# geek-ai/MAgent

Hardware: NVIDIA B200
Metric: agent-steps/sec on battle map at 1/2/4/8 B200 vs ref C++ on host cores (higher is better)
Workload: dtype f32

## Files before the change

magent_b200/csrc/backend_cuda.cu:

```cuda
#include <cooperative_groups.h>
#include <cuda_runtime.h>
#include <cuda_fp16.h>
#include <stdio.h>
#include <stdlib.h>
#include <string>
#include <string.h>
#include <atomic>
#include <mutex>
#include <vector>

#include "backend.h"
#if defined(MG_PHASE_TIMING)
namespace mg { __device__ long long mg_phase_clock[8 * 32]; }
#endif
#include "obs_phases.h"

namespace cg = cooperative_groups;

namespace mg {
[[noreturn]] void fatal(const char *fmt, ...);
namespace be {

#define CUDA_CHECK(expr)                                                                          \
    do {                                                                                          \
        cudaError_t _e = (expr);                                                                  \
        if (_e != cudaSuccess) mg::fatal("CUDA error %s at %s:%d (%s)", cudaGetErrorString(_e),   \
                                         __FILE__, __LINE__, #expr);                              \
    } while (0)

static std::atomic<long long> g_launches{0};

enum { ATTR_STEP = 0, ATTR_OBS0 = 1, ATTR_N = 1 + 8, ATTR_MAX_DEVICES = 64 };
static std::mutex g_attr_mu;
static size_t g_attr_smem[ATTR_MAX_DEVICES][ATTR_N];
template <class K>
static void ensure_dynamic_smem(int device, int slot, K kernel, size_t smem) {
    std::lock_guard<std::mutex> lk(g_attr_mu);
    size_t &have = g_attr_smem[device % ATTR_MAX_DEVICES][slot];
    if (smem <= have) return;
    CUDA_CHECK(cudaFuncSetAttribute(kernel, cudaFuncAttributeMaxDynamicSharedMemorySize, (int)smem));
    have = smem;
}

struct Ctx {
    int device = 0, sms = 0;
    cudaStream_t stream = nullptr;
    cudaStream_t copy = nullptr;
    cudaEvent_t ev_wire = nullptr, ev_done = nullptr;
    bool profile = false;
    std::vector<cudaEvent_t> events;
    size_t events_used = 0;
    float *mm_pad = nullptr; size_t mm_pad_n = 0; int mm_stride = 0;
    int4 *obs_hdr = nullptr; size_t obs_hdr_n = 0;
    struct ObsCfg { size_t smem = (size_t)-1; int ctas_per_sm = 1; } obs_cfg[8];
    int *pin_done = nullptr; size_t pin_done_n = 0;
    int *pin_counts = nullptr; size_t pin_counts_n = 0;
    cudaEvent_t ev_counts = nullptr;
    WireMark *wire_slots = nullptr; size_t wire_slots_n = 0;
    WireMark *wire_stream = nullptr; size_t wire_stream_n = 0;
    WireHdr *wire_hdr = nullptr; size_t wire_hdr_n = 0;
    long long *wire_base = nullptr; size_t wire_base_n = 0;
    int *wire_chunk_total = nullptr;
    WireHdr *h_wire_hdr = nullptr; size_t h_wire_hdr_n = 0;
    WireMark *h_wire_marks = nullptr; size_t h_wire_marks_n = 0;
    long long *h_wire_base = nullptr; size_t h_wire_base_n = 0;
    float *h_mm = nullptr; size_t h_mm_n = 0;
    std::vector<cudaEvent_t> wave_events;
    int waves_queued = 0;
    std::vector<cudaEvent_t> dma_events; size_t dma_head = 0, dma_tail = 0;
    bool capturing = false;
    std::vector<cudaGraphExec_t> graphs;
};

static void no_capture(const Ctx *c, const char *what) {
    if (c->capturing) mg::fatal("%s is not possible while a CUDA graph is being captured (run one un-captured step first so that "
                                "every buffer has its size)", what);
}

struct DeviceGuard {
    explicit DeviceGuard(const Ctx *c) { int cur = -1; cudaGetDevice(&cur); if (cur != c->device) CUDA_CHECK(cudaSetDevice(c->device)); }
};

const char *name() { return "cuda-sm_100a"; }

#if defined(MG_PHASE_TIMING)
extern "C" __attribute__((visibility("default"))) void magent_b200_debug_phase_clocks(long long *out) {
    CUDA_CHECK(cudaMemcpyFromSymbol(out, mg::mg_phase_clock, sizeof(long long) * 8 * 32));
}
#endif

int device_count() {
    int n = 0;
    if (cudaGetDeviceCount(&n) != cudaSuccess) { cudaGetLastError(); return 0; }
    return n;
}

Ctx *create(int device, std::string *err) {
    int n = device_count();
    if (n <= 0) { if (err) *err = "cudaGetDeviceCount found no device"; return nullptr; }
    if (device < 0) {
        if (cudaGetDevice(&device) != cudaSuccess) device = 0;
    }
    if (device >= n) { if (err) *err = "device_id out of range"; return nullptr; }
    cudaError_t e = cudaSetDevice(device);
    if (e != cudaSuccess) { if (err) *err = cudaGetErrorString(e); return nullptr; }
    cudaDeviceProp prop;
    CUDA_CHECK(cudaGetDeviceProperties(&prop, device));
    Ctx *c = new Ctx();
    c->device = device;
    c->sms = prop.multiProcessorCount;
    CUDA_CHECK(cudaStreamCreate(&c->stream));
    CUDA_CHECK(cudaStreamCreateWithFlags(&c->copy, cudaStreamNonBlocking));
    CUDA_CHECK(cudaEventCreateWithFlags(&c->ev_wire, cudaEventDisableTiming));
    CUDA_CHECK(cudaEventCreateWithFlags(&c->ev_done, cudaEventDisableTiming));
    CUDA_CHECK(cudaEventCreateWithFlags(&c->ev_counts, cudaEventDisableTiming));
    return c;
}
void destroy(Ctx *c) {
    if (!c) return;
    cudaSetDevice(c->device);
    for (cudaGraphExec_t e : c->graphs) if (e) cudaGraphExecDestroy(e);
    cudaStreamSynchronize(c->stream); cudaStreamSynchronize(c->copy);
    for (cudaEvent_t e : c->events) cudaEventDestroy(e);
    for (cudaEvent_t e : c->wave_events) cudaEventDestroy(e);
    for (cudaEvent_t e : c->dma_events) cudaEventDestroy(e);
    cudaEventDestroy(c->ev_wire); cudaEventDestroy(c->ev_done);
    cudaFree(c->mm_pad); cudaFree(c->obs_hdr);
    cudaFree(c->wire_slots); cudaFree(c->wire_stream); cudaFree(c->wire_hdr); cudaFree(c->wire_base); cudaFree(c->wire_chunk_total);
    cudaEventDestroy(c->ev_counts); cudaFreeHost(c->pin_counts);
    cudaFreeHost(c->pin_done); cudaFreeHost(c->h_wire_hdr); cudaFreeHost(c->h_wire_marks); cudaFreeHost(c->h_wire_base); cudaFreeHost(c->h_mm);
    cudaStreamDestroy(c->stream); cudaStreamDestroy(c->copy);
    delete c;
}
int device_of(const Ctx *c) { return c->device; }
int sm_count(const Ctx *c) { return c->sms; }
void *stream_handle(const Ctx *c) { return (void *)c->stream; }

void *dmalloc(Ctx *c, size_t bytes) { no_capture(c, "a device allocation"); DeviceGuard g(c); void *p = nullptr; CUDA_CHECK(cudaMalloc(&p, bytes ? bytes : 16)); return p; }
void dfree(Ctx *c, void *p) { if (p) { DeviceGuard g(c); cudaFree(p); } }
void dmemset(Ctx *c, void *p, int byte, size_t bytes) { DeviceGuard g(c); CUDA_CHECK(cudaMemsetAsync(p, byte, bytes, c->stream)); }
void h2d(Ctx *c, void *dst, const void *src, size_t bytes) {
    if (!bytes) return;
    no_capture(c, "a blocking host-to-device copy");
    DeviceGuard g(c);
    CUDA_CHECK(cudaMemcpyAsync(dst, src, bytes, cudaMemcpyHostToDevice, c->stream));
    CUDA_CHECK(cudaStreamSynchronize(c->stream));
}
void d2h(Ctx *c, void *dst, const void *src, size_t bytes) {
    if (!bytes) return;
    no_capture(c, "a blocking device-to-host copy");
    DeviceGuard g(c);
    CUDA_CHECK(cudaMemcpyAsync(dst, src, bytes, cudaMemcpyDeviceToHost, c->stream));
    CUDA_CHECK(cudaStreamSynchronize(c->stream));
}
void d2d(Ctx *c, void *dst, const void *src, size_t bytes) {
    if (!bytes) return;
    DeviceGuard g(c);
    CUDA_CHECK(cudaMemcpyAsync(dst, src, bytes, cudaMemcpyDeviceToDevice, c->stream));
}
void *host_alloc(size_t bytes) {
    void *p = nullptr;
    if (cudaHostAlloc(&p, bytes ? bytes : 16, cudaHostAllocPortable) != cudaSuccess) { cudaGetLastError(); return nullptr; }
    return p;
}
void host_free(void *p) { if (p) cudaFreeHost(p); }
bool host_register(void *p, size_t bytes) {
    if (cudaHostRegister(p, bytes, cudaHostRegisterPortable) != cudaSuccess) { cudaGetLastError(); return false; }
    return true;
}
void host_unregister(void *p) { if (cudaHostUnregister(p) != cudaSuccess) cudaGetLastError(); }
bool is_device_ptr(const void *p) {
    if (!p) return false;
    cudaPointerAttributes at;
    if (cudaPointerGetAttributes(&at, p) != cudaSuccess) { cudaGetLastError(); return false; }
    return at.type == cudaMemoryTypeDevice || at.type == cudaMemoryTypeManaged;
}
bool is_pinned_host_ptr(const void *p) {
    if (!p) return false;
    cudaPointerAttributes at;
    if (cudaPointerGetAttributes(&at, p) != cudaSuccess) { cudaGetLastError(); return false; }
    return at.type == cudaMemoryTypeHost;
}
void sync(Ctx *c) { no_capture(c, "a synchronisation"); DeviceGuard g(c); CUDA_CHECK(cudaStreamSynchronize(c->stream)); CUDA_CHECK(cudaStreamSynchronize(c->copy)); }
long long launch_count() { return g_launches.load(); }
void profile_enable(Ctx *c, bool on) { c->profile = on; c->events_used = 0; }
static void profile_pair(Ctx *c, cudaEvent_t *e0, cudaEvent_t *e1) {
    if (c->events_used + 2 > c->events.size()) {
        for (int i = 0; i < 64; ++i) { cudaEvent_t e; CUDA_CHECK(cudaEventCreate(&e)); c->events.push_back(e); }
    }
    *e0 = c->events[c->events_used]; *e1 = c->events[c->events_used + 1];
    c->events_used += 2;
}
void profile_read(Ctx *c, double *ms, long long *n) {
    DeviceGuard g(c);
    double total = 0.0;
    for (size_t i = 0; i + 1 < c->events_used; i += 2) {
        CUDA_CHECK(cudaEventSynchronize(c->events[i + 1]));
        float t = 0;
        CUDA_CHECK(cudaEventElapsedTime(&t, c->events[i], c->events[i + 1]));
        total += t;
    }
    *ms = total; *n = (long long)(c->events_used / 2);
}

bool capture_begin(Ctx *c) {
    DeviceGuard guard(c);
    CUDA_CHECK(cudaStreamSynchronize(c->stream));
    CUDA_CHECK(cudaStreamBeginCapture(c->stream, cudaStreamCaptureModeRelaxed));
    c->capturing = true;
    return true;
}
int capture_end(Ctx *c) {
    DeviceGuard guard(c);
    cudaGraph_t g = nullptr;
    c->capturing = false;
    CUDA_CHECK(cudaStreamEndCapture(c->stream, &g));
    cudaGraphExec_t exec = nullptr;
    CUDA_CHECK(cudaGraphInstantiate(&exec, g, 0));
    CUDA_CHECK(cudaGraphDestroy(g));
    c->graphs.push_back(exec);
    return (int)c->graphs.size() - 1;
}
bool capturing(const Ctx *c) { return c->capturing; }
void graph_launch(Ctx *c, int id) {
    DeviceGuard guard(c);
    if (id < 0 || id >= (int)c->graphs.size() || !c->graphs[id]) mg::fatal("invalid graph id %d", id);
    CUDA_CHECK(cudaGraphLaunch(c->graphs[id], c->stream));
}
void graph_destroy_all(Ctx *c) {
    DeviceGuard guard(c);
    for (cudaGraphExec_t e : c->graphs) if (e) cudaGraphExecDestroy(e);
    c->graphs.clear();
}

static void post_launch(const char *what) {
    ++g_launches;
    cudaError_t e = cudaGetLastError();
    if (e != cudaSuccess) mg::fatal("kernel launch failed (%s): %s", what, cudaGetErrorString(e));
}

__device__ __forceinline__ int block_excl_scan(int v, int &total) {
    __shared__ int warp_sums[32];
    __shared__ int block_total;
    const int lane = threadIdx.x & 31, wid = threadIdx.x >> 5, nw = (blockDim.x + 31) >> 5;
    int incl = v;
#pragma unroll
    for (int d = 1; d < 32; d <<= 1) {
        int t = __shfl_up_sync(0xffffffffu, incl, d);
        if (lane >= d) incl += t;
    }
    if (lane == 31) warp_sums[wid] = incl;
    __syncthreads();
    if (wid == 0) {
        int w = lane < nw ? warp_sums[lane] : 0;
        int wi = w;
#pragma unroll
        for (int d = 1; d < 32; d <<= 1) {
            int t = __shfl_up_sync(0xffffffffu, wi, d);
            if (lane >= d) wi += t;
        }
        if (lane < nw) warp_sums[lane] = wi - w;
        if (lane == 31) block_total = wi;
    }
    __syncthreads();
    int excl = incl - v + warp_sums[wid];
    total = block_total;
    __syncthreads();
    return excl;
}

struct CtaCtx {
    GroupEnum *enum_smem;
    MG_HD GroupEnum *enums() { return enum_smem; }
    MG_HD bool is_cta_leader() const {
#if defined(__CUDA_ARCH__)
        return threadIdx.x == 0;
#else
        return true;
#endif
    }
    MG_HD void sync_cta() {
#if defined(__CUDA_ARCH__)
        __syncthreads();
#endif
    }
    int *flag_smem;
    MG_HD int *flags(ArenaHdr *) { return flag_smem; }
    int cnt[MG_N_COUNTERS];
    MG_HD void add_count(const EngineDev &, int kind, long long v) { cnt[kind] += (int)v; }
    int *cnt_smem;
    MG_HD void flush_counts(const EngineDev &E) {
#if defined(__CUDA_ARCH__)
#pragma unroll
        for (int k = 0; k < MG_N_COUNTERS; ++k) {
            int v = cnt[k];
            cnt[k] = 0;
#pragma unroll
            for (int d = 16; d > 0; d >>= 1) v += __shfl_xor_sync(0xffffffffu, v, d);
            if (v && (threadIdx.x & 31) == 0) atomicAdd(&cnt_smem[k], v);
        }
        __syncthreads();
        if (threadIdx.x < MG_N_COUNTERS) {
            const int v = cnt_smem[threadIdx.x];
            cnt_smem[threadIdx.x] = 0;
            if (v) atomicAdd((unsigned long long *)&E.counters[threadIdx.x], (unsigned long long)v);
        }
#endif
    }
    MG_HD int tid() const {
#if defined(__CUDA_ARCH__)
        return threadIdx.x;
#else
        return 0;
#endif
    }
    MG_HD int nth() const {
#if defined(__CUDA_ARCH__)
        return blockDim.x;
#else
        return 1;
#endif
    }
    MG_HD void sync() {
#if defined(__CUDA_ARCH__)
        __syncthreads();
#endif
    }
    template <class P, class Em>
    MG_HD int scan(int n, P pred, Em emit) {
#if defined(__CUDA_ARCH__)
        int running = 0;
        for (int tile = 0; tile < n; tile += blockDim.x) {
            int i = tile + threadIdx.x;
            int p = i < n ? pred(i) : 0;
            int tot;
            int ex = block_excl_scan(p, tot);
            if (p) emit(i, running + ex);
            running += tot;
        }
        return running;
#else
        return 0;
#endif
    }
};

struct GridCtx {
    GroupEnum *enum_smem;
    MG_HD GroupEnum *enums() { return enum_smem; }
    MG_HD bool is_cta_leader() const {
#if defined(__CUDA_ARCH__)
        return threadIdx.x == 0;
#else
        return true;
#endif
    }
    MG_HD void sync_cta() {
#if defined(__CUDA_ARCH__)
        __syncthreads();
#endif
    }
    int *scratch;
    int parity;
    MG_HD int *flags(ArenaHdr *hdr) { return hdr->changed; }
    int cnt[MG_N_COUNTERS];
    MG_HD void add_count(const EngineDev &, int kind, long long v) { cnt[kind] += (int)v; }
    MG_HD void flush_counts(const EngineDev &E) {
#if defined(__CUDA_ARCH__)
#pragma unroll
        for (int k = 0; k < MG_N_COUNTERS; ++k) {
            int v = cnt[k];
            cnt[k] = 0;
#pragma unroll
            for (int d = 16; d > 0; d >>= 1) v += __shfl_xor_sync(0xffffffffu, v, d);
            if (v && (threadIdx.x & 31) == 0) atomicAdd((unsigned long long *)&E.counters[k], (unsigned long long)v);
        }
#endif
    }
    MG_HD int tid() const {
#if defined(__CUDA_ARCH__)
        return blockIdx.x * blockDim.x + threadIdx.x;
#else
        return 0;
#endif
    }
    MG_HD int nth() const {
#if defined(__CUDA_ARCH__)
        return gridDim.x * blockDim.x;
#else
        return 1;
#endif
    }
    MG_HD void sync() {
#if defined(__CUDA_ARCH__)
        cg::this_grid().sync();
#endif
    }
    template <class P, class Em>
    MG_HD int scan(int n, P pred, Em emit) {
#if defined(__CUDA_ARCH__)
        const int nb = gridDim.x, bid = blockIdx.x;
        const int L = (n + nb - 1) / nb;
        const int lo = min(n, bid * L), hi = min(n, lo + L);
        int cnt = 0;
        for (int i = lo + threadIdx.x; i < hi; i += blockDim.x) cnt += pred(i);
        int cta_total;
        block_excl_scan(cnt, cta_total);
        int *sc = scratch + (parity & 1) * 4096;
        parity ^= 1;
        if (threadIdx.x == 0) sc[bid] = cta_total;
        cg::this_grid().sync();
        int below = 0, all = 0;
        for (int b = threadIdx.x; b < nb; b += blockDim.x) { int v = sc[b]; all += v; if (b < bid) below += v; }
        int base, total;
        block_excl_scan(below, base);
        block_excl_scan(all, total);
        int running = base;
        for (int tile = lo; tile < hi; tile += blockDim.x) {
            int i = tile + threadIdx.x;
            int p = i < hi ? pred(i) : 0;
            int tot;
            int ex = block_excl_scan(p, tot);
            if (p) emit(i, running + ex);
            running += tot;
        }
        return total;
#else
        return 0;
#endif
    }
};

__device__ __forceinline__ void load_engine(EngineDev *sE, const EngineDev *gE) {
    const int *src = (const int *)gE;
    int *dst = (int *)sE;
    for (int i = threadIdx.x; i < (int)(sizeof(EngineDev) / sizeof(int)); i += blockDim.x) dst[i] = src[i];
    __syncthreads();
}

constexpr int STEP_THREADS = 1024;
constexpr int GRID_THREADS = 512;

static size_t step_scratch_bytes(int cap_total, int max_body) {
    return (size_t)cap_total * (9 * 4 + 4 * (size_t)max_body) + (((size_t)cap_total + 15) & ~(size_t)15);
}

__device__ __forceinline__ void step_scratch_to_smem(EngineDev *sE, unsigned char *base) {
    const size_t n = (size_t)sE->cap_total;
    int *p = (int *)base;
    sE->att_rank = p; p += n;  sE->tgt = p; p += n;       sE->in_head = p; p += n;  sE->in_next = p; p += n;
    sE->death = p; p += n;
    sE->mv_nx = p; sE->jv = p; p += n;
    sE->mv_ny = p; sE->sh_head = p; p += n;
    sE->mv_key = (unsigned *)p; sE->sh_next = p; p += n;
    sE->hp_fin = (float *)p; sE->att_agent = p; p += n;
    sE->cl_next = p; sE->sh_first = p; p += n * sE->max_body;
    sE->mv_state = (unsigned char *)p;
    sE->scratch_stride = 0;
}

__global__ void __launch_bounds__(STEP_THREADS) step_kernel_cta(const EngineDev *gE, StepArgs S, int scratch_in_smem) {
    extern __shared__ __align__(16) unsigned char step_smem[];
    __shared__ EngineDev sE;
    load_engine(&sE, gE);
    if (scratch_in_smem) {
        if (threadIdx.x == 0) step_scratch_to_smem(&sE, step_smem);
        __syncthreads();
    }
    __shared__ int relax_flags[3];
    __shared__ int counter_sums[MG_N_COUNTERS];
    __shared__ GroupEnum enum_store[2];
    if (threadIdx.x < MG_N_COUNTERS) counter_sums[threadIdx.x] = 0;
    CtaCtx c;
    c.flag_smem = relax_flags;
    c.cnt_smem = counter_sums;
    c.enum_smem = enum_store;
    for (int k = 0; k < MG_N_COUNTERS; ++k) c.cnt[k] = 0;
    for (int a = blockIdx.x; a < sE.A; a += gridDim.x) run_step(c, sE, S, a);
}

__global__ void __launch_bounds__(STEP_THREADS) step_kernel_grid(const EngineDev *gE, StepArgs S) {
    __shared__ EngineDev sE;
    load_engine(&sE, gE);
    __shared__ GroupEnum enum_store[2];
    GridCtx c;
    c.scratch = sE.team_scratch;
    c.parity = 0;
    c.enum_smem = enum_store;
    for (int k = 0; k < MG_N_COUNTERS; ++k) c.cnt[k] = 0;
    for (int a = 0; a < sE.A; ++a) run_step(c, sE, S, a);
}

__global__ void __launch_bounds__(STEP_THREADS) cull_kernel_cta(const EngineDev *gE, unsigned curmask) {
    __shared__ EngineDev sE;
    load_engine(&sE, gE);
    CtaCtx c;
    c.flag_smem = nullptr;
    c.cnt_smem = nullptr;
    c.enum_smem = nullptr;
    for (int a = blockIdx.x; a < sE.A; a += gridDim.x) run_cull(c, sE, curmask, a);
}

__global__ void __launch_bounds__(STEP_THREADS) cull_kernel_grid(const EngineDev *gE, unsigned curmask) {
    __shared__ EngineDev sE;
    load_engine(&sE, gE);
    GridCtx c;
    c.scratch = sE.team_scratch;
    c.parity = 0;
    c.enum_smem = nullptr;
    for (int a = 0; a < sE.A; ++a) run_cull(c, sE, curmask, a);
}

static const int GRID_MODE_THRESHOLD = 32768;

static int step_block_size(int sms, int arenas, int max_agents) {
    if (arenas >= 2 * sms) return 256;
    if (max_agents >= 768) return 1024;
    return max_agents >= 384 ? 512 : 256;
}

static int coop_grid(const Ctx *c, const void *kernel) {
    int per_sm = 0;
    CUDA_CHECK(cudaOccupancyMaxActiveBlocksPerMultiprocessor(&per_sm, kernel, GRID_THREADS, 0));
    if (per_sm < 1) mg::fatal("cooperative kernel does not fit on an SM");
    int g = per_sm * c->sms;
    return g > 4096 ? 4096 : g;
}

void launch_step(Ctx *c, const EngineDev *dE, const EngineDev &hE, const StepArgs &S, int max_agents) {
    DeviceGuard guard(c);
    const int g_sms = c->sms;
    if (max_agents > GRID_MODE_THRESHOLD) {
        int grid = coop_grid(c, (const void *)step_kernel_grid);
        StepArgs s = S;
        void *args[] = {(void *)&dE, (void *)&s};
        CUDA_CHECK(cudaLaunchCooperativeKernel((const void *)step_kernel_grid, dim3(grid), dim3(GRID_THREADS), args, 0, c->stream));
        post_launch("step_kernel_grid");
    } else {
        const size_t sbytes = step_scratch_bytes(hE.cap_total, hE.max_body);
        static const int smem_pref = getenv("MAGENT_B200_STEP_SMEM") ? atoi(getenv("MAGENT_B200_STEP_SMEM")) : -1;
        const bool in_smem = sbytes <= 200 * 1024 && smem_pref != 0;
        int threads = step_block_size(g_sms, hE.A, max_agents);
        size_t smem = 0;
        if (in_smem) {
            smem = sbytes;
            threads = max_agents >= 768 ? (hE.A > g_sms ? 512 : 1024) : (max_agents >= 384 ? 512 : 256);
            ensure_dynamic_smem(c->device, ATTR_STEP, step_kernel_cta, smem);
        }
        static const int threads_pref = getenv("MAGENT_B200_STEP_THREADS") ? atoi(getenv("MAGENT_B200_STEP_THREADS")) : 0;
        if (threads_pref >= 32 && threads_pref <= STEP_THREADS) threads = threads_pref & ~31;
        int per_sm = 1;
        CUDA_CHECK(cudaOccupancyMaxActiveBlocksPerMultiprocessor(&per_sm, step_kernel_cta, threads, smem));
        if (per_sm < 1) per_sm = 1;
        int grid = hE.A < per_sm * g_sms ? hE.A : per_sm * g_sms;
        step_kernel_cta<<<grid, threads, smem, c->stream>>>(dE, S, in_smem ? 1 : 0);
        post_launch("step_kernel_cta");
    }
}

void launch_cull(Ctx *c, const EngineDev *dE, const EngineDev &hE, unsigned curmask, int max_agents) {
    DeviceGuard guard(c);
    const int g_sms = c->sms;
    if (max_agents > GRID_MODE_THRESHOLD) {
        int grid = coop_grid(c, (const void *)cull_kernel_grid);
        void *args[] = {(void *)&dE, (void *)&curmask};
        CUDA_CHECK(cudaLaunchCooperativeKernel((const void *)cull_kernel_grid, dim3(grid), dim3(GRID_THREADS), args, 0, c->stream));
        post_launch("cull_kernel_grid");
    } else {
        int grid = hE.A < 8 * g_sms ? hE.A : 8 * g_sms;
        static const int cull_pref = getenv("MAGENT_B200_CULL_THREADS") ? atoi(getenv("MAGENT_B200_CULL_THREADS")) : 0;
        int threads = max_agents >= 768 ? 512 : step_block_size(g_sms, hE.A, max_agents);
        if (cull_pref >= 32 && cull_pref <= STEP_THREADS) threads = cull_pref & ~31;
        cull_kernel_cta<<<grid, threads, 0, c->stream>>>(dE, curmask);
        post_launch("cull_kernel_cta");
    }
}

__global__ void __launch_bounds__(1024) offsets_kernel(const EngineDev *gE) {
    const int g = blockIdx.x;
    const int A = gE->A;
    const int *n = gE->n + (size_t)g * A;
    int *off = gE->off + (size_t)g * (A + 1);
    int running = 0;
    for (int tile = 0; tile < A; tile += blockDim.x) {
        int a = tile + threadIdx.x;
        int v = a < A ? n[a] : 0;
        int tot;
        int ex = block_excl_scan(v, tot);
        if (a < A) off[a] = running + ex;
        running += tot;
    }
    if (threadIdx.x == 0) off[A] = running;
}

void launch_offsets(Ctx *c, const EngineDev *dE, const EngineDev &hE) {
    DeviceGuard guard(c);
    offsets_kernel<<<hE.G, 1024, 0, c->stream>>>(dE);
    post_launch("offsets_kernel");
}

__device__ __forceinline__ int locate_arena(const int *off, int A, int idx) {
    int lo = 0, hi = A;
    while (hi - lo > 1) {
        int mid = (lo + hi) >> 1;
        if (off[mid] <= idx) lo = mid; else hi = mid;
    }
    return lo;
}

__global__ void __launch_bounds__(256) info_kernel(const EngineDev *gE, unsigned curmask, int kind, int g,
                                                   void *buf, int n_total, int chunks_per_arena) {
    const EngineDev &E = *gE;
    const int *off = E.off + (size_t)g * (E.A + 1);
    const AgentSoA &s = E.grp[g].soa[(curmask >> g) & 1u];
    const int a = blockIdx.x / chunks_per_arena;
    const int i = (blockIdx.x - a * chunks_per_arena) * blockDim.x + threadIdx.x;
    const int o0 = off[a];
    const int o = o0 + i;
    if (i < off[a + 1] - o0 && o < n_total) {
        const long gi = (long)a * E.grp[g].cap + i;
        switch (kind) {
            case INFO_ID: ((int *)buf)[o] = s.id[gi]; break;
            case INFO_POS: ((int2 *)buf)[o] = make_int2(s.x[gi], s.y[gi]); break;
            case INFO_ALIVE: ((unsigned char *)buf)[o] = (s.flags[gi] & FLAG_DEAD) ? 0 : 1; break;
            case INFO_REWARD: ((float *)buf)[o] = s.next_reward[gi] + E.hdr[a].grp_reward[g]; break;
            case INFO_HP: ((float *)buf)[o] = s.hp[gi]; break;
            case INFO_ACTION_SCATTER: s.act[gi] = ((const int *)buf)[o]; break;
        }
    }
}

void launch_info(Ctx *c, const EngineDev *dE, const EngineDev &hE, unsigned curmask, int kind, int group, void *buf, int n_total) {
    DeviceGuard guard(c);
    const int cap = hE.grp[group].cap;
    const int threads = cap >= 256 ? 256 : ((cap + 31) & ~31);
    const int cpa = (cap + threads - 1) / threads;
    info_kernel<<<(unsigned)((size_t)hE.A * cpa), threads, 0, c->stream>>>(dE, curmask, kind, group, buf, n_total, cpa);
    post_launch("info_kernel");
}

__device__ __forceinline__ unsigned long long splitmix64(unsigned long long x) {
    x += 0x9E3779B97F4A7C15ull;
    x = (x ^ (x >> 30)) * 0xBF58476D1CE4E5B9ull;
    x = (x ^ (x >> 27)) * 0x94D049BB133111EBull;
    return x ^ (x >> 31);
}

__global__ void __launch_bounds__(256) random_actions_kernel(const EngineDev *gE, unsigned curmask, int g,
                                                             unsigned long long seed, int n_total, int chunks_per_arena) {
    const EngineDev &E = *gE;
    const int *off = E.off + (size_t)g * (E.A + 1);
    const AgentSoA &s = E.grp[g].soa[(curmask >> g) & 1u];
    const unsigned na = (unsigned)E.grp[g].n_action;
    seed += (unsigned long long)E.counters[CNT_STEPS] * 0xA24BAED4963EE407ull;
    const int a = blockIdx.x / chunks_per_arena;
    const int i = (blockIdx.x - a * chunks_per_arena) * blockDim.x + threadIdx.x;
    const int o0 = off[a];
    const int o = o0 + i;
    if (i < off[a + 1] - o0 && o < n_total)
        s.act[(long)a * E.grp[g].cap + i] = (int)((splitmix64(seed ^ ((unsigned long long)o * 0xD1342543DE82EF95ull)) >> 33) % na);
}

void launch_random_actions(Ctx *c, const EngineDev *dE, const EngineDev &hE, unsigned curmask, int group,
                           unsigned long long seed, int n_total) {
    DeviceGuard guard(c);
    const int cap = hE.grp[group].cap;
    const int threads = cap >= 256 ? 256 : ((cap + 31) & ~31);
    const int cpa = (cap + threads - 1) / threads;
    random_actions_kernel<<<(unsigned)((size_t)hE.A * cpa), threads, 0, c->stream>>>(dE, curmask, group, seed, n_total, cpa);
    post_launch("random_actions_kernel");
}

__global__ void __launch_bounds__(256) minimap_small_kernel(const EngineDev *gE, unsigned curmask, int og, float *mm_val, int stride) {
    extern __shared__ int hist[];
    __shared__ int counted_s;
    const EngineDev &E = *gE;
    const int ag = blockIdx.x;
    const int a = ag / E.G, j = ag - a * E.G;
    const int vw = E.grp[og].view_w, vh = E.grp[og].view_h, cells = vw * vh;
    const int n = E.n[j * E.A + a];
    for (int k = threadIdx.x; k < cells; k += blockDim.x) hist[k] = 0;
    if (threadIdx.x == 0) counted_s = 0;
    __syncthreads();
    const GroupDev &G = E.grp[j];
    const AgentSoA &s = G.soa[(curmask >> j) & 1u];
    const int scale_h = (E.H + vh - 1) / vh, scale_w = (E.W + vw - 1) / vw;
    const bool skip_absorbed = E.grp[og].can_absorb != 0;
    int counted = 0;
    for (int i = threadIdx.x; i < n; i += blockDim.x) {
        const long gi = (long)a * G.cap + i;
        if (skip_absorbed && (s.flags[gi] & FLAG_ABSORBED)) continue;
        atomicAdd(&hist[(s.y[gi] / scale_h) * vw + s.x[gi] / scale_w], 1);
        ++counted;
    }
#pragma unroll
    for (int d = 16; d > 0; d >>= 1) counted += __shfl_xor_sync(0xffffffffu, counted, d);
    if ((threadIdx.x & 31) == 0 && counted) atomicAdd(&counted_s, counted);
    __syncthreads();
    const int tot = counted_s;
    float *out = mm_val + (size_t)a * stride + (size_t)j * cells;
    for (int k = threadIdx.x; k < cells; k += blockDim.x)
        out[k] = tot ? (float)hist[k] / (float)tot : __int_as_float((int)0xFFC00000u);
}

__global__ void __launch_bounds__(256) obs_prepare_kernel(const EngineDev *gE, unsigned curmask, int og, int chunk) {
    extern __shared__ int hist[];
    const EngineDev &E = *gE;
    const int ag = blockIdx.y;
    const int a = ag / E.G, j = ag - a * E.G;
    const int vw = E.grp[og].view_w, vh = E.grp[og].view_h, cells = vw * vh;
    const int n = E.n[j * E.A + a];
    const int lo = blockIdx.x * chunk;
    if (lo >= n) return;
    const int hi = min(n, lo + chunk);
    for (int k = threadIdx.x; k < cells; k += blockDim.x) hist[k] = 0;
    __syncthreads();
    const GroupDev &G = E.grp[j];
    const AgentSoA &s = G.soa[(curmask >> j) & 1u];
    const int scale_h = (E.H + vh - 1) / vh, scale_w = (E.W + vw - 1) / vw;
    const bool skip_absorbed = E.grp[og].can_absorb != 0;
    int counted = 0;
    for (int i = lo + threadIdx.x; i < hi; i += blockDim.x) {
        long gi = (long)a * G.cap + i;
        if (skip_absorbed && (s.flags[gi] & FLAG_ABSORBED)) continue;
        atomicAdd(&hist[(s.y[gi] / scale_h) * vw + s.x[gi] / scale_w], 1);
        ++counted;
    }
    if (counted) atomicAdd(&E.mm_total[ag], counted);
    __syncthreads();
    int *out = E.mm_count + (size_t)ag * cells;
    for (int k = threadIdx.x; k < cells; k += blockDim.x)
        if (hist[k]) atomicAdd(&out[k], hist[k]);
}

__global__ void __launch_bounds__(256) minimap_norm_kernel(const EngineDev *gE, int og, float *mm_val, int total, int stride) {
    const EngineDev &E = *gE;
    const int cells = E.grp[og].view_w * E.grp[og].view_h;
    for (int k = blockIdx.x * blockDim.x + threadIdx.x; k < total; k += gridDim.x * blockDim.x) {
        int ag = k / cells;
        const int tot = E.mm_total[ag];
        const int a = ag / E.G;
        mm_val[(size_t)a * stride + (k - a * E.G * cells)] = tot ? (float)E.mm_count[k] / (float)tot : __int_as_float((int)0xFFC00000u);
    }
}

void launch_obs_prepare(Ctx *c, const EngineDev *dE, const EngineDev &hE, unsigned curmask, int og, float *mm_val) {
    if (!mm_val) return;
    DeviceGuard guard(c);
    const int g_sms = c->sms;
    const int cells = hE.grp[og].view_w * hE.grp[og].view_h;
    const int total = hE.A * hE.G * cells;
    int cap_max = 0;
    for (int g = 0; g < hE.G; ++g) cap_max = cap_max > hE.grp[g].cap ? cap_max : hE.grp[g].cap;
    c->mm_stride = (hE.G * cells + 3) & ~3;
    const size_t need = (size_t)hE.A * c->mm_stride;
    if (need > c->mm_pad_n) {
        no_capture(c, "growing the minimap buffer");
        if (c->mm_pad) { CUDA_CHECK(cudaStreamSynchronize(c->stream)); CUDA_CHECK(cudaStreamSynchronize(c->copy)); cudaFree(c->mm_pad); }
        CUDA_CHECK(cudaMalloc(&c->mm_pad, need * sizeof(float)));
        CUDA_CHECK(cudaMemsetAsync(c->mm_pad, 0, need * sizeof(float), c->stream));
        c->mm_pad_n = need;
    }
    if (cap_max <= 8192 && (size_t)cells * sizeof(int) <= 48 * 1024) {
        minimap_small_kernel<<<hE.A * hE.G, 256, cells * sizeof(int), c->stream>>>(dE, curmask, og, c->mm_pad, c->mm_stride);
        post_launch("minimap_small_kernel");
        return;
    }
    CUDA_CHECK(cudaMemsetAsync(hE.mm_count, 0, (size_t)total * 4, c->stream));
    CUDA_CHECK(cudaMemsetAsync(hE.mm_total, 0, (size_t)hE.A * hE.G * 4, c->stream));
    const int chunk = 4096;
    dim3 grid((cap_max + chunk - 1) / chunk, hE.A * hE.G);
    obs_prepare_kernel<<<grid, 256, cells * sizeof(int), c->stream>>>(dE, curmask, og, chunk);
    post_launch("obs_prepare_kernel");
    int g2 = (total + 255) / 256;
    if (g2 > 8 * g_sms) g2 = 8 * g_sms;
    minimap_norm_kernel<<<g2, 256, 0, c->stream>>>(dE, og, c->mm_pad, total, c->mm_stride);
    post_launch("minimap_norm_kernel");
}

#ifndef OBS_TA_N
#define OBS_TA_N 4
#endif
#ifndef OBS_ABLATE
#define OBS_ABLATE 0
#endif

template <typename T> struct ObsOut;
template <> struct ObsOut<float> {
    static constexpr int TA = OBS_TA_N;
    static __device__ __forceinline__ float cv(float v) { return v; }
};
template <> struct ObsOut<__half> {
    static constexpr int TA = 2 * OBS_TA_N;
    static __device__ __forceinline__ __half cv(float v) {
        if (v != v) {
            const unsigned u = __float_as_uint(v);
            unsigned short r = (unsigned short)(0x7c00u + ((u & 0x7fffffu) >> 13));
            if (r == 0x7c00u) ++r;
            return __ushort_as_half((unsigned short)(r | ((u >> 16) & 0x8000u)));
        }
        return __float2half_rn(v);
    }
};

struct ObsParams {
    int A, W, H, G, C;
    int vw, vh, cells, rec, F;
    int ox, oy;
    int scale_w, scale_h, minimap;
    int cap, embedding, n_action, n_total;
    const unsigned char *mask;
    const int *off;
    const unsigned char *kind_plane;
    const float *hpn_plane;
    int kpad, kw;
    long kplane;
    int chunk;
    int turn, body_w, body_l;
    const unsigned char *dir;
    const int *x, *y, *id, *act;
    const float *last_reward;
    const float *mm;
    int mm_stride;
    const int4 *hdr;
    void *view, *feature;
    int mm_ch[MG_MAX_GROUPS];
    int grp_ch[MG_MAX_GROUPS];
};

__device__ __forceinline__ uint32_t smem_u32(const void *p) { return (uint32_t)__cvta_generic_to_shared(p); }

template <typename T>
__global__ void __launch_bounds__(256) obs_headers_kernel(ObsParams P, int4 *hdr, int chunks_per_arena) {
    extern __shared__ __align__(16) unsigned char hdr_smem[];
    T *rows = (T *)hdr_smem;
    const int a = blockIdx.x / chunks_per_arena;
    const int i0 = (blockIdx.x - a * chunks_per_arena) * blockDim.x;
    const int o0 = P.off[a], n_a = P.off[a + 1] - o0;
    if (i0 >= n_a) return;
    int cnt = min((int)blockDim.x, n_a - i0);
    cnt = min(cnt, P.n_total - (o0 + i0));
    if (cnt <= 0) return;
    const int total = cnt * P.F;
    for (int q = threadIdx.x; q < total; q += blockDim.x) rows[q] = ObsOut<T>::cv(0.0f);
    __syncthreads();
    if ((int)threadIdx.x < cnt) {
        const int i = i0 + threadIdx.x;
        const long gi = (long)a * P.cap + i;
        const int x = P.x[gi], y = P.y[gi];
        const int self_cell = P.minimap ? (y / P.scale_h) * P.vw + x / P.scale_w : -1;
        const int heading = P.turn ? (int)P.dir[gi] : 0;
        hdr[o0 + i] = make_int4(x, y, a, (self_cell & 0xffff) | (heading << 16));
        T *f = rows + (size_t)threadIdx.x * P.F;
        unsigned id = (unsigned)P.id[gi];
        const int nbits = min(P.embedding, 31);
        id &= nbits >= 32 ? 0xffffffffu : ((1u << nbits) - 1u);
        while (id) {
            const int bit = __ffs(id) - 1;
            f[bit] = ObsOut<T>::cv(1.0f);
            id &= id - 1;
        }
        T *g = f + P.embedding;
        const int act = P.act[gi];
        if (act >= 0 && act < P.n_action) g[act] = ObsOut<T>::cv(1.0f);
        g[P.n_action] = ObsOut<T>::cv(P.last_reward[gi]);
        if (P.minimap) {
            g[P.n_action + 1] = ObsOut<T>::cv((float)x / (float)P.W);
            g[P.n_action + 2] = ObsOut<T>::cv((float)y / (float)P.H);
        }
    }
    __syncthreads();
    T *out = (T *)P.feature + (size_t)(o0 + i0) * P.F;
    if (sizeof(T) == 4 && ((((size_t)out) & 15) == 0)) {
        const int v4 = total >> 2;
        for (int q = threadIdx.x; q < v4; q += blockDim.x) ((float4 *)out)[q] = ((const float4 *)rows)[q];
        for (int q = (v4 << 2) + threadIdx.x; q < total; q += blockDim.x) out[q] = rows[q];
    } else {
        for (int q = threadIdx.x; q < total; q += blockDim.x) out[q] = rows[q];
    }
}

#ifndef OBS_MIN_CTAS
#define OBS_MIN_CTAS 8
#endif
#ifndef OBS_CHUNK
#define OBS_CHUNK 4
#endif
template <typename T, int NIT, bool TURN>
__global__ void __launch_bounds__(32 * ObsOut<T>::TA, OBS_MIN_CTAS * OBS_TA_N / ObsOut<T>::TA)
obs_render_kernel(const __grid_constant__ ObsParams P) {
    const int n_total = min(P.n_total, __ldg(P.off + P.A));
    constexpr int OBS_TA = ObsOut<T>::TA;
    constexpr int OBS_THREADS = 32 * OBS_TA;
    extern __shared__ __align__(128) unsigned char smem_raw[];
    T *buf = (T *)smem_raw;
    int2 *lut = (int2 *)(buf + OBS_TA * P.rec);
    __shared__ int n_in_s;
    const int lane = threadIdx.x & 31, warp = threadIdx.x >> 5;

    const int lut_stride = (P.cells + 1) & ~1;
    if (warp == 0) {
        int k = 0;
        for (int base = 0; base < P.cells; base += 32) {
            const int cell = base + lane;
            const bool in = cell < P.cells && P.mask[cell];
            const unsigned bal = __ballot_sync(0xffffffffu, in);
            if (in) {
                const int vy = cell / P.vw, vx = cell - vy * P.vw;
                const int q = k + __popc(bal & ((1u << lane) - 1u));
                if (!TURN) lut[q] = make_int2(cell * P.C, (P.oy + vy) * P.kw + P.ox + vx);
                else {
                    for (int d = 0; d < 4; ++d) {
                        int rx = 0, ry = 0, dx, dy;
                        if (d == DIR_SOUTH) { rx = P.body_w - 1; ry = P.body_l - 1; }
                        else if (d == DIR_WEST) ry = P.body_w - 1;
                        else if (d == DIR_EAST) rx = P.body_l - 1;
                        const int ex = P.ox + vx, ey = P.oy + vy;
                        if (d == DIR_NORTH) { dx = ex; dy = ey; }
                        else if (d == DIR_SOUTH) { dx = -ex; dy = -ey; }
                        else if (d == DIR_WEST) { dx = ey; dy = -ex; }
                        else { dx = -ey; dy = ex; }
                        lut[d * lut_stride + q] = make_int2(cell * P.C, (ry + dy) * P.kw + rx + dx);
                    }
                }
            }
            k += __popc(bal);
        }
        if (lane == 0) n_in_s = k;
    }
    __syncthreads();
    const int n_in = n_in_s;
    const int n_tiles = (n_total + OBS_TA - 1) / OBS_TA;
    constexpr bool LUT_REGS = NIT <= 4 && !TURN;
    int2 lreg[LUT_REGS ? NIT : 1];
    if (LUT_REGS) {
#pragma unroll
        for (int it = 0; it < (LUT_REGS ? NIT : 1); ++it) lreg[it] = it * 32 + lane < n_in ? lut[it * 32 + lane] : make_int2(-1, 0);
    }
    auto lutv = [&](int it, int hd) -> int2 {
        if (TURN) return it * 32 + lane < n_in ? lut[hd * lut_stride + it * 32 + lane] : make_int2(-1, 0);
        return LUT_REGS ? lreg[LUT_REGS ? it : 0] : (it * 32 + lane < n_in ? lut[it * 32 + lane] : make_int2(-1, 0));
    };
    auto plane_base = [&](const int4 &h) -> long { return h.z * P.kplane + (long)(h.y + P.kpad) * P.kw + h.x + P.kpad; };

    auto load_kinds = [&](const int4 &h, bool on, int (&kd)[NIT]) {
        const unsigned char *kp = P.kind_plane + plane_base(h);
        const int hd = TURN ? (h.w >> 16) & 3 : 0;
#pragma unroll
        for (int it = 0; it < NIT; ++it) {
            const int2 l = lutv(it, hd);
            kd[it] = (on && l.x >= 0 && !(OBS_ABLATE & 1)) ? __ldg(kp + l.y) : 0;
        }
    };
    unsigned long long chpack = 0ull;
#pragma unroll
    for (int j = 0; j < MG_MAX_GROUPS; ++j) chpack |= (unsigned long long)(P.grp_ch[j] & 0xff) << (8 * j);
    auto mark = [&](T *px, int t, float hp, bool on) {
        const bool agent = kind_is_agent(t);
        const int ch = agent ? (int)((chpack >> (8 * kind_group(t))) & 0xffull) : (t == KIND_FOOD ? 1 : 0);
        px[ch] = ObsOut<T>::cv(on ? 1.0f : 0.0f);
        if (agent) px[ch + 1] = ObsOut<T>::cv(on ? hp : 0.0f);
    };

    const int chunk = P.chunk;
    const int chunk_jump = ((int)gridDim.x - 1) * chunk;
    auto next_tile = [&](int t) -> int { return ((t + 1) % chunk) ? t + 1 : t + 1 + chunk_jump; };
    int tile = blockIdx.x * chunk;
    int tile1 = next_tile(tile), tile2 = next_tile(tile1);
    const int tile_end = n_tiles;
    const int4 zero4 = make_int4(0, 0, 0, 0);
    int4 hA = zero4, hA1 = zero4;
    int kind[NIT];
    int rec_arena = -1, prev_hd = 0, prev_self = -1;
    unsigned prev_kinds[(NIT + 3) / 4];
#pragma unroll
    for (int q = 0; q < (NIT + 3) / 4; ++q) prev_kinds[q] = 0u;
    float self_orig = 0.0f;
    bool prev_tail = false;
    {
        const int o0 = tile * OBS_TA + warp, o1 = tile1 * OBS_TA + warp;
        const bool on0 = tile < tile_end && o0 < n_total;
        if (on0) hA = P.hdr[o0];
        if (o1 < n_total) hA1 = P.hdr[o1];
        load_kinds(hA, on0, kind);
    }
    for (; tile < tile_end; tile = tile1, tile1 = tile2, tile2 = next_tile(tile2)) {
        const int t0 = tile * OBS_TA;
        const int cnt = min(OBS_TA, n_total - t0);
        const bool active = warp < cnt;
        const int a = hA.z;
        const float *hpnp = P.hpn_plane + plane_base(hA);
        const int hd = TURN ? (hA.w >> 16) & 3 : 0;
        float thp[NIT];
#pragma unroll
        for (int it = 0; it < NIT; ++it) {
            thp[it] = 0.0f;
            if (kind_is_agent(kind[it])) thp[it] = (kind[it] & KIND_FULL) ? 1.0f : __ldg(hpnp + lutv(it, hd).y);
        }
        int kind1[NIT];
        const long o1 = (long)tile1 * OBS_TA + warp;
        load_kinds(hA1, o1 < n_total, kind1);
        int4 hA2 = zero4;
        {
            const long o2 = (long)tile2 * OBS_TA + warp;
            if (o2 < n_total) hA2 = P.hdr[o2];
        }
        if (threadIdx.x == 0) asm volatile("cp.async.bulk.wait_group.read 0;" ::: "memory");
        __syncthreads();
        if (active && !(OBS_ABLATE & 2)) {
            T *dst = buf + warp * P.rec;
            const int self = (int)(short)(hA.w & 0xffff);
            if (a != rec_arena) {
                if (sizeof(T) == 4) {
                    float *w = (float *)dst;
                    const int n = P.rec;
                    const int head = min(n, (int)((4u - ((unsigned)(warp * P.rec) & 3u)) & 3u));
                    const int body = (n - head) >> 2;
                    if (lane < head) w[lane] = 0.0f;
                    float4 *w4 = (float4 *)(w + head);
                    const float4 z = make_float4(0.f, 0.f, 0.f, 0.f);
                    for (int q = lane; q < body; q += 32) w4[q] = z;
                    const int tail0 = head + (body << 2);
                    if (tail0 + lane < n) w[tail0 + lane] = 0.0f;
                } else {
                    for (int q = lane; q < P.rec; q += 32) dst[q] = ObsOut<T>::cv(0.0f);
                }
                __syncwarp();
                if (P.minimap) {
                    const float *rows = P.mm + (size_t)a * P.mm_stride;
                    for (int j = 0; j < P.G; ++j) {
                        T *d = dst + P.mm_ch[j];
                        for (int cell = lane; cell < P.cells; cell += 32) d[cell * P.C] = ObsOut<T>::cv(__ldg(rows + j * P.cells + cell));
                    }
                }
                rec_arena = a;
                __syncwarp();
            } else {
#pragma unroll
                for (int it = 0; it < NIT; ++it) {
                    const int t = (prev_kinds[it >> 2] >> ((it & 3) * 8)) & 0xff;
                    if (t != 0) mark(dst + lutv(it, prev_hd).x, t, 0.0f, false);
                }
                if (prev_tail) {
                    for (int k = NIT * 32 + lane; k < n_in; k += 32) {
                        T *px = dst + lut[(TURN ? prev_hd * lut_stride : 0) + k].x;
                        for (int ch = 0; ch < P.C; ++ch) {
                            bool mm_ch = false;
                            for (int j = 0; j < P.G; ++j) mm_ch |= P.minimap && ch == P.mm_ch[j];
                            if (!mm_ch) px[ch] = ObsOut<T>::cv(0.0f);
                        }
                    }
                }
                if (P.minimap && lane < P.G && prev_self >= 0) dst[prev_self * P.C + P.mm_ch[lane]] = ObsOut<T>::cv(self_orig);
                __syncwarp();
            }
            if (P.minimap && lane < P.G) {
                const float v = __ldg(P.mm + (size_t)a * P.mm_stride + lane * P.cells + self);
                self_orig = v;
                if (v == v) dst[self * P.C + P.mm_ch[lane]] = ObsOut<T>::cv(v + 1.0f);
            }
            prev_self = self;
            prev_hd = hd;
#pragma unroll
            for (int q = 0; q < (NIT + 3) / 4; ++q) prev_kinds[q] = 0u;
#pragma unroll
            for (int it = 0; it < NIT; ++it) {
                const int t = kind[it];
                prev_kinds[it >> 2] |= (unsigned)t << ((it & 3) * 8);
                if (t != 0) mark(dst + lutv(it, hd).x, t, thp[it], true);
            }
            prev_tail = false;
            const unsigned char *kindp = P.kind_plane + plane_base(hA);
            for (int k = NIT * 32 + lane; k < n_in; k += 32) {
                const int2 l = lut[(TURN ? hd * lut_stride : 0) + k];
                const int t = __ldg(kindp + l.y);
                if (t != 0) { mark(dst + l.x, t, kind_is_agent(t) ? ((t & KIND_FULL) ? 1.0f : __ldg(hpnp + l.y)) : 0.0f, true); }
                prev_tail = true;
            }
        }
        asm volatile("fence.proxy.async.shared::cta;" ::: "memory");
        __syncthreads();
        T *gout = (T *)P.view + (size_t)t0 * P.rec;
        const unsigned bytes = (unsigned)cnt * (unsigned)P.rec * (unsigned)sizeof(T);
        if ((bytes & 15u) == 0 && (((size_t)gout) & 15) == 0) {
            if (threadIdx.x == 0 && !(OBS_ABLATE & 8)) {
                asm volatile("cp.async.bulk.global.shared::cta.bulk_group [%0], [%1], %2;"
                             :: "l"(gout), "r"(smem_u32(buf)), "r"(bytes) : "memory");
                asm volatile("cp.async.bulk.commit_group;" ::: "memory");
            }
        } else {
            for (int q = threadIdx.x; q < cnt * P.rec; q += OBS_THREADS) gout[q] = buf[q];
            __syncthreads();
        }
        hA = hA1; hA1 = hA2;
#pragma unroll
        for (int it = 0; it < NIT; ++it) kind[it] = kind1[it];
    }
    if (threadIdx.x == 0) asm volatile("cp.async.bulk.wait_group 0;" ::: "memory");
}

template <typename T, int NIT, bool TURN>
static void launch_obs_typed(Ctx *c, int cfg_slot, const EngineDev &hE, ObsParams &P, int n_total,
                             bool with_headers = true, bool headers_only = false) {
    const int g_sms = c->sms;
    constexpr int TA = ObsOut<T>::TA;
    constexpr int THREADS = 32 * TA;
    const size_t tile_bytes = (size_t)TA * P.rec * sizeof(T);
    const size_t smem = tile_bytes + (size_t)(P.turn ? 4 : 1) * ((P.cells + 1) & ~1) * sizeof(int2);
    if (smem > 227 * 1024) mg::fatal("observation record too large for the render kernel (%zu bytes of shared memory)", smem);
    const int tiles = (n_total + TA - 1) / TA;
    if ((size_t)n_total > c->obs_hdr_n) {
        no_capture(c, "growing the observation header table");
        if (c->obs_hdr) { CUDA_CHECK(cudaStreamSynchronize(c->stream)); cudaFree(c->obs_hdr); }
        c->obs_hdr_n = (size_t)n_total + n_total / 4 + 64;
        CUDA_CHECK(cudaMalloc(&c->obs_hdr, c->obs_hdr_n * sizeof(int4)));
    }
    P.hdr = c->obs_hdr;
    if (with_headers) {
        int threads = 256;
        while (threads > 32 && (size_t)threads * P.F * sizeof(T) > 48 * 1024) threads >>= 1;
        const size_t hsm = (size_t)threads * P.F * sizeof(T);
        if (hsm > 48 * 1024) mg::fatal("feature row too long for the header kernel (%d elements)", P.F);
        const int cpa = (P.cap + threads - 1) / threads;
        obs_headers_kernel<T><<<(unsigned)((size_t)P.A * cpa), threads, hsm, c->stream>>>(P, c->obs_hdr, cpa);
        post_launch("obs_headers_kernel");
    }
    if (headers_only) return;
    Ctx::ObsCfg &cfg = c->obs_cfg[cfg_slot];
    ensure_dynamic_smem(c->device, ATTR_OBS0 + cfg_slot, obs_render_kernel<T, NIT, TURN>, smem);
    if (smem != cfg.smem) {
        CUDA_CHECK(cudaOccupancyMaxActiveBlocksPerMultiprocessor(&cfg.ctas_per_sm, obs_render_kernel<T, NIT, TURN>, THREADS, smem));
        if (cfg.ctas_per_sm < 1) cfg.ctas_per_sm = 1;
        cfg.smem = smem;
    }
    const int ctas_per_sm = cfg.ctas_per_sm;
    const int grid = tiles < ctas_per_sm * g_sms ? tiles : ctas_per_sm * g_sms;
    P.chunk = tiles / (ctas_per_sm * g_sms);
    if (P.chunk < 1) P.chunk = 1;
    const int max_chunk = sizeof(T) == 2 ? 2 * OBS_CHUNK : OBS_CHUNK;
    if (P.chunk > max_chunk) P.chunk = max_chunk;
    cudaEvent_t e0 = nullptr, e1 = nullptr;
    const bool timed = c->profile && !c->capturing;
    if (timed) { profile_pair(c, &e0, &e1); CUDA_CHECK(cudaEventRecord(e0, c->stream)); }
    obs_render_kernel<T, NIT, TURN><<<grid, THREADS, smem, c->stream>>>(P);
    post_launch("obs_render_kernel");
    if (timed) CUDA_CHECK(cudaEventRecord(e1, c->stream));
}

static void fill_obs_params(Ctx *c, const EngineDev &hE, const ObsArgs &O, const float *mm_val, int n_total, ObsParams &P) {
    const int g = O.group;
    const GroupDev &G = hE.grp[g];
    memset(&P, 0, sizeof P);
    P.A = hE.A; P.W = hE.W; P.H = hE.H; P.G = hE.G; P.C = hE.n_channel;
    P.vw = G.view_w; P.vh = G.view_h; P.cells = G.view_w * G.view_h; P.rec = P.cells * P.C; P.F = G.feature_size;
    P.ox = G.view_xoff + G.view_x1; P.oy = G.view_yoff + G.view_y1;
    P.scale_w = (hE.W + G.view_w - 1) / G.view_w; P.scale_h = (hE.H + G.view_h - 1) / G.view_h;
    P.minimap = mm_val != nullptr;
    P.cap = G.cap; P.embedding = hE.embedding_size; P.n_action = G.n_action; P.n_total = n_total;
    P.mask = G.view_mask;
    P.off = hE.off + (size_t)g * (hE.A + 1);
    P.kind_plane = hE.kind; P.hpn_plane = hE.hpn; P.kpad = hE.kpad; P.kw = hE.kw; P.kplane = hE.kplane;
    const AgentSoA &s = G.soa[(O.curmask >> g) & 1u];
    P.x = s.x; P.y = s.y; P.id = s.id; P.act = s.act; P.last_reward = s.last_reward; P.dir = s.dir;
    P.turn = hE.turn_mode; P.body_w = G.body_w; P.body_l = G.body_l;
    P.mm = mm_val ? c->mm_pad : nullptr; P.mm_stride = mm_val ? c->mm_stride : 0;
    P.view = O.view; P.feature = O.feature;
    const int stride = 2 + (hE.minimap_mode ? 1 : 0);
    for (int j = 0; j < hE.G; ++j) {
        int rel = j - g; if (rel < 0) rel += hE.G;
        const int ch = hE.channel_base + rel * stride;
        P.mm_ch[j] = ch + 2;
        P.grp_ch[j] = ch;
    }
}

static void launch_obs_dispatch(Ctx *c, const EngineDev &hE, const ObsArgs &O, ObsParams &P, int n_total, bool with_headers, bool headers_only) {
    const bool small_view = hE.grp[O.group].view_count <= 4 * 32;
    if (hE.turn_mode) {
        if (O.half) launch_obs_typed<__half, 8, true>(c, 0, hE, P, n_total, with_headers, headers_only);
        else launch_obs_typed<float, 8, true>(c, 1, hE, P, n_total, with_headers, headers_only);
    } else if (O.half) {
        if (small_view) launch_obs_typed<__half, 4, false>(c, 2, hE, P, n_total, with_headers, headers_only);
        else launch_obs_typed<__half, 8, false>(c, 3, hE, P, n_total, with_headers, headers_only);
    } else {
        if (small_view) launch_obs_typed<float, 4, false>(c, 4, hE, P, n_total, with_headers, headers_only);
        else launch_obs_typed<float, 8, false>(c, 5, hE, P, n_total, with_headers, headers_only);
    }
}

void launch_obs(Ctx *c, const EngineDev *, const EngineDev &hE, const ObsArgs &O, const float *mm_val, int n_total) {
    DeviceGuard guard(c);
    ObsParams P;
    fill_obs_params(c, hE, O, mm_val, n_total, P);
    launch_obs_dispatch(c, hE, O, P, n_total, true, false);
}

__global__ void __launch_bounds__(256) done_reduce_kernel(const EngineDev *gE, int *out) {
    __shared__ int all_s;
    if (threadIdx.x == 0) all_s = 1;
    __syncthreads();
    int all = 1;
    for (int a = threadIdx.x; a < gE->A; a += blockDim.x) all &= gE->done[a] & 1;
    if (!all) all_s = 0;
    __syncthreads();
    if (threadIdx.x == 0) *out = all_s;
}

void read_done(Ctx *c, const EngineDev &hE, int *done_words) {
    no_capture(c, "env_step with a host `done`");
    DeviceGuard guard(c);
    if ((size_t)hE.A > c->pin_done_n) {
        if (c->pin_done) cudaFreeHost(c->pin_done);
        c->pin_done_n = (size_t)hE.A + 64;
        CUDA_CHECK(cudaHostAlloc((void **)&c->pin_done, c->pin_done_n * sizeof(int), cudaHostAllocDefault));
    }
    CUDA_CHECK(cudaMemcpyAsync(c->pin_done, hE.done, (size_t)hE.A * sizeof(int), cudaMemcpyDeviceToHost, c->stream));
    CUDA_CHECK(cudaStreamSynchronize(c->stream));
    memcpy(done_words, c->pin_done, (size_t)hE.A * sizeof(int));
}

void counts_fetch_begin(Ctx *c, const int *dev_off, size_t n_ints) {
    no_capture(c, "the asynchronous count fetch");
    DeviceGuard guard(c);
    if (n_ints > c->pin_counts_n) {
        if (c->pin_counts) { CUDA_CHECK(cudaStreamSynchronize(c->stream)); cudaFreeHost(c->pin_counts); }
        c->pin_counts_n = n_ints + 64;
        CUDA_CHECK(cudaHostAlloc((void **)&c->pin_counts, c->pin_counts_n * sizeof(int), cudaHostAllocDefault));
    }
    CUDA_CHECK(cudaMemcpyAsync(c->pin_counts, dev_off, n_ints * sizeof(int), cudaMemcpyDeviceToHost, c->stream));
    CUDA_CHECK(cudaEventRecord(c->ev_counts, c->stream));
}
const int *counts_fetch_wait(Ctx *c) {
    DeviceGuard guard(c);
    CUDA_CHECK(cudaEventSynchronize(c->ev_counts));
    return c->pin_counts;
}

void launch_done_to_device(Ctx *c, const EngineDev *dE, const EngineDev &, int *dev_done) {
    DeviceGuard guard(c);
    done_reduce_kernel<<<1, 256, 0, c->stream>>>(dE, dev_done);
    post_launch("done_reduce_kernel");
}

__global__ void __launch_bounds__(256) obs_wire_kernel(const __grid_constant__ ObsParams P, WireHdr *whdr, WireMark *slots,
                                                       int slot_stride, int *chunk_total) {
    extern __shared__ __align__(16) unsigned char wire_smem[];
    int2 *lut = (int2 *)wire_smem;
    __shared__ int n_in_s;
    const int lane = threadIdx.x & 31, warp = threadIdx.x >> 5;
    const int lut_stride = (P.cells + 1) & ~1;
    if (warp == 0) {
        int k = 0;
        for (int base = 0; base < P.cells; base += 32) {
            const int cell = base + lane;
            const bool in = cell < P.cells && P.mask[cell];
            const unsigned bal = __ballot_sync(0xffffffffu, in);
            if (in) {
                const int vy = cell / P.vw, vx = cell - vy * P.vw;
                const int q = k + __popc(bal & ((1u << lane) - 1u));
                if (!P.turn) lut[q] = make_int2(cell * P.C, (P.oy + vy) * P.kw + P.ox + vx);
                else {
                    for (int d = 0; d < 4; ++d) {
                        int rx = 0, ry = 0, dx, dy;
                        if (d == DIR_SOUTH) { rx = P.body_w - 1; ry = P.body_l - 1; }
                        else if (d == DIR_WEST) ry = P.body_w - 1;
                        else if (d == DIR_EAST) rx = P.body_l - 1;
                        const int ex = P.ox + vx, ey = P.oy + vy;
                        if (d == DIR_NORTH) { dx = ex; dy = ey; }
                        else if (d == DIR_SOUTH) { dx = -ex; dy = -ey; }
                        else if (d == DIR_WEST) { dx = ey; dy = -ex; }
                        else { dx = -ey; dy = ex; }
                        lut[d * lut_stride + q] = make_int2(cell * P.C, (ry + dy) * P.kw + rx + dx);
                    }
                }
            }
            k += __popc(bal);
        }
        if (lane == 0) n_in_s = k;
    }
    __syncthreads();
    const int n_in = n_in_s;
    const int warps = gridDim.x * (blockDim.x >> 5);
    for (int o = blockIdx.x * (blockDim.x >> 5) + warp; o < P.n_total; o += warps) {
        const int4 h = P.hdr[o];
        const long pb = h.z * P.kplane + (long)(h.y + P.kpad) * P.kw + h.x + P.kpad;
        const unsigned char *kp = P.kind_plane + pb;
        const float *hpnp = P.hpn_plane + pb;
        const int2 *l = lut + (P.turn ? ((h.w >> 16) & 3) * lut_stride : 0);
        WireMark *row = slots + (size_t)o * slot_stride;
        int running = 0;
        for (int base = 0; base < n_in; base += 32) {
            const int k = base + lane;
            int t = 0;
            int2 lk = make_int2(0, 0);
            if (k < n_in) { lk = l[k]; t = __ldg(kp + lk.y); }
            const unsigned bal = __ballot_sync(0xffffffffu, t != 0);
            if (t != 0) {
                WireMark m;
                if (t == KIND_WALL) { m.off = (unsigned)lk.x; m.val = 0.0f; }
                else if (t == KIND_FOOD) { m.off = (unsigned)lk.x + 1u; m.val = 0.0f; }
                else { m.off = (unsigned)(lk.x + P.grp_ch[kind_group(t)]) | WIRE_HAS_HP; m.val = (t & KIND_FULL) ? 1.0f : __ldg(hpnp + lk.y); }
                row[running + __popc(bal & ((1u << lane) - 1u))] = m;
            }
            running += __popc(bal);
        }
        if (lane == 0) {
            WireHdr w;
            w.arena = h.z;
            w.self_cell = (unsigned short)(h.w & 0xffff);
            w.count = (unsigned short)running;
            whdr[o] = w;
            if (running) atomicAdd(&chunk_total[o / WIRE_CHUNK], running);
        }
    }
}

__global__ void __launch_bounds__(1024) wire_scan_kernel(const int *chunk_total, long long *base, int n_chunks) {
    __shared__ long long carry_s;
    if (threadIdx.x == 0) carry_s = 0;
    __syncthreads();
    for (int tile = 0; tile < n_chunks; tile += blockDim.x) {
        const int cidx = tile + threadIdx.x;
        const int v = cidx < n_chunks ? chunk_total[cidx] : 0;
        int tot;
        const int ex = block_excl_scan(v, tot);
        const long long carry = carry_s;
        if (cidx < n_chunks) base[cidx] = carry + ex;
        __syncthreads();
        if (threadIdx.x == 0) carry_s = carry + tot;
        __syncthreads();
    }
    if (threadIdx.x == 0) base[n_chunks] = carry_s;
}

__global__ void __launch_bounds__(256) wire_compact_kernel(const WireHdr *whdr, const WireMark *slots, int slot_stride,
                                                           const long long *base, WireMark *stream, int n_total, int n_chunks) {
    __shared__ int off_s[WIRE_CHUNK];
    __shared__ unsigned short cnt_s[WIRE_CHUNK];
    const int lane = threadIdx.x & 31, warp = threadIdx.x >> 5, nw = blockDim.x >> 5;
    for (int ch = blockIdx.x; ch < n_chunks; ch += gridDim.x) {
        const int o0 = ch * WIRE_CHUNK, cnt_obs = min(WIRE_CHUNK, n_total - o0);
        int running = 0;
        for (int tile = 0; tile < WIRE_CHUNK; tile += blockDim.x) {
            const int i = tile + threadIdx.x;
            const int v = i < cnt_obs ? (int)whdr[o0 + i].count : 0;
            int tot;
            const int ex = block_excl_scan(v, tot);
            off_s[i] = running + ex;
            cnt_s[i] = (unsigned short)v;
            running += tot;
        }
        __syncthreads();
        WireMark *dst = stream + base[ch];
        for (int i = warp; i < cnt_obs; i += nw) {
            const int n = cnt_s[i], off = off_s[i];
            const WireMark *src = slots + (size_t)(o0 + i) * slot_stride;
            for (int k = lane; k < n; k += 32) dst[off + k] = src[k];
        }
        __syncthreads();
    }
}

template <class T>
static void grow_dev(Ctx *c, T *&p, size_t &have, size_t need) {
    if (need <= have) return;
    if (p) { CUDA_CHECK(cudaStreamSynchronize(c->stream)); CUDA_CHECK(cudaStreamSynchronize(c->copy)); cudaFree(p); }
    have = need + need / 4 + 64;
    CUDA_CHECK(cudaMalloc((void **)&p, have * sizeof(T)));
}
template <class T>
static void grow_pinned(Ctx *c, T *&p, size_t &have, size_t need) {
    if (need <= have) return;
    if (p) { CUDA_CHECK(cudaStreamSynchronize(c->copy)); cudaFreeHost(p); }
    have = need + need / 2 + 1024;
    CUDA_CHECK(cudaHostAlloc((void **)&p, have * sizeof(T), cudaHostAllocDefault));
}

void obs_wire_begin(Ctx *c, const EngineDev *, const EngineDev &hE, const ObsArgs &O, const float *mm_val, int n_total,
                    WireDesc *out) {
    no_capture(c, "an observation into host memory");
    DeviceGuard guard(c);
    ObsParams P;
    fill_obs_params(c, hE, O, mm_val, n_total, P);
    launch_obs_dispatch(c, hE, O, P, n_total, true, true);
    const int n_in = hE.grp[O.group].view_count;
    const int n_chunks = (n_total + WIRE_CHUNK - 1) / WIRE_CHUNK;
    grow_dev(c, c->wire_slots, c->wire_slots_n, (size_t)n_total * n_in);
    grow_dev(c, c->wire_hdr, c->wire_hdr_n, (size_t)n_total);
    {
        size_t have = c->wire_base_n;
        grow_dev(c, c->wire_base, c->wire_base_n, (size_t)n_chunks + 1);
        if (c->wire_base_n != have) {
            if (c->wire_chunk_total) cudaFree(c->wire_chunk_total);
            CUDA_CHECK(cudaMalloc((void **)&c->wire_chunk_total, c->wire_base_n * sizeof(int)));
        }
    }
    CUDA_CHECK(cudaMemsetAsync(c->wire_chunk_total, 0, (size_t)n_chunks * sizeof(int), c->stream));
    {
        const size_t smem = (size_t)(P.turn ? 4 : 1) * ((P.cells + 1) & ~1) * sizeof(int2);
        if (smem > 48 * 1024) mg::fatal("view too large for the wire kernel (%zu bytes of shared memory)", smem);
        int grid = (n_total + 7) / 8;
        if (grid > 8 * c->sms) grid = 8 * c->sms;
        obs_wire_kernel<<<grid, 256, smem, c->stream>>>(P, c->wire_hdr, c->wire_slots, n_in, c->wire_chunk_total);
        post_launch("obs_wire_kernel");
        wire_scan_kernel<<<1, 1024, 0, c->stream>>>(c->wire_chunk_total, c->wire_base, n_chunks);
        post_launch("wire_scan_kernel");
    }
    grow_pinned(c, c->h_wire_base, c->h_wire_base_n, (size_t)n_chunks + 1);
    CUDA_CHECK(cudaMemcpyAsync(c->h_wire_base, c->wire_base, ((size_t)n_chunks + 1) * sizeof(long long), cudaMemcpyDeviceToHost, c->stream));
    CUDA_CHECK(cudaEventRecord(c->ev_done, c->stream));
    if (mm_val) {
        grow_pinned(c, c->h_mm, c->h_mm_n, (size_t)hE.A * c->mm_stride);
        CUDA_CHECK(cudaMemcpyAsync(c->h_mm, c->mm_pad, (size_t)hE.A * c->mm_stride * sizeof(float), cudaMemcpyDeviceToHost, c->stream));
    }
    grow_pinned(c, c->h_wire_hdr, c->h_wire_hdr_n, (size_t)n_total);
    CUDA_CHECK(cudaEventSynchronize(c->ev_done));
    const long long total_marks = c->h_wire_base[n_chunks];
    grow_dev(c, c->wire_stream, c->wire_stream_n, (size_t)total_marks + 1);
    grow_pinned(c, c->h_wire_marks, c->h_wire_marks_n, (size_t)total_marks + 1);
    {
        int grid = n_chunks < 8 * c->sms ? n_chunks : 8 * c->sms;
        wire_compact_kernel<<<grid, 256, 0, c->stream>>>(c->wire_hdr, c->wire_slots, n_in, c->wire_base, c->wire_stream, n_total, n_chunks);
        post_launch("wire_compact_kernel");
    }
    CUDA_CHECK(cudaEventRecord(c->ev_wire, c->stream));
    CUDA_CHECK(cudaStreamWaitEvent(c->copy, c->ev_wire, 0));
    int cpw = (n_chunks + 7) / 8;
    if (cpw < 4) cpw = 4;
    const int n_waves = (n_chunks + cpw - 1) / cpw;
    while ((int)c->wave_events.size() < n_waves) {
        cudaEvent_t e; CUDA_CHECK(cudaEventCreateWithFlags(&e, cudaEventDisableTiming)); c->wave_events.push_back(e);
    }
    for (int q = 0; q < n_waves; ++q) {
        const int half = (n_waves + 1) / 2;
        const int w = (q & 1) ? half + (q >> 1) : (q >> 1);
        out->wave_order[q] = w;
        const int c0 = w * cpw, c1 = (c0 + cpw < n_chunks) ? c0 + cpw : n_chunks;
        const size_t o0 = (size_t)c0 * WIRE_CHUNK, o1 = (size_t)c1 * WIRE_CHUNK < (size_t)n_total ? (size_t)c1 * WIRE_CHUNK : (size_t)n_total;
        CUDA_CHECK(cudaMemcpyAsync(c->h_wire_hdr + o0, c->wire_hdr + o0, (o1 - o0) * sizeof(WireHdr), cudaMemcpyDeviceToHost, c->copy));
        const long long m0 = c->h_wire_base[c0], m1 = c->h_wire_base[c1];
        if (m1 > m0) CUDA_CHECK(cudaMemcpyAsync(c->h_wire_marks + m0, c->wire_stream + m0, (size_t)(m1 - m0) * sizeof(WireMark), cudaMemcpyDeviceToHost, c->copy));
        CUDA_CHECK(cudaEventRecord(c->wave_events[w], c->copy));
    }
    c->waves_queued = n_waves;
    out->hdr = c->h_wire_hdr; out->marks = c->h_wire_marks; out->chunk_base = c->h_wire_base;
    out->mm = mm_val ? c->h_mm : nullptr; out->mm_stride = mm_val ? c->mm_stride : 0;
    out->n_total = n_total; out->n_chunks = n_chunks; out->n_waves = n_waves; out->chunks_per_wave = cpw;
}

void obs_wire_wait(Ctx *c, int wave) {
    DeviceGuard guard(c);
    CUDA_CHECK(cudaEventSynchronize(c->wave_events[wave]));
}

void dma_d2h_async(Ctx *c, void *dst, const void *src, size_t bytes) {
    DeviceGuard guard(c);
    CUDA_CHECK(cudaMemcpyAsync(dst, src, bytes, cudaMemcpyDeviceToHost, c->copy));
    if (c->dma_events.size() < 64) {
        while (c->dma_events.size() < 64) { cudaEvent_t e; CUDA_CHECK(cudaEventCreateWithFlags(&e, cudaEventDisableTiming)); c->dma_events.push_back(e); }
    }
    if (c->dma_tail - c->dma_head >= c->dma_events.size()) {
        CUDA_CHECK(cudaEventSynchronize(c->dma_events[c->dma_head % c->dma_events.size()]));
        ++c->dma_head;
    }
    CUDA_CHECK(cudaEventRecord(c->dma_events[c->dma_tail % c->dma_events.size()], c->copy));
    ++c->dma_tail;
}

void dma_wait(Ctx *c, int keep_in_flight) {
    DeviceGuard guard(c);
    while ((long long)(c->dma_tail - c->dma_head) > (long long)keep_in_flight) {
        CUDA_CHECK(cudaEventSynchronize(c->dma_events[c->dma_head % c->dma_events.size()]));
        ++c->dma_head;
    }
}

}
}
```

magent_b200/csrc/dev_types.h:

```cpp
#pragma once
#include <stdint.h>
#include "hd.h"

namespace mg {

enum { MG_MAX_GROUPS = 8, MG_MAX_RULES = 64, MG_MAX_PROG = 16, MG_MAX_RECV = 4, MG_MAX_IN = 4, MG_MAX_ALLQ = 16 };
enum { MG_N_COUNTERS = 8 };
enum Counter { CNT_AGENT_STEPS = 0, CNT_ATTACKS, CNT_HITS, CNT_KILLS, CNT_STARVED,
               CNT_MOVES_OK, CNT_MOVES_BLOCKED, CNT_STEPS };

enum : int { OCC_EMPTY = -1, OCC_WALL = -2, OCC_FOOD = -3 };
enum : int { TGT_NONE = -1, TGT_FOOD = -3 };
enum : int { KIND_EMPTY = 0, KIND_WALL = 1, KIND_GROUP0 = 2, KIND_FOOD = 255 };
enum : int { KIND_FULL = 0x40, KIND_GROUP_MASK = 0x3f };
MG_HD unsigned char kind_agent(int g, bool full_hp) { return (unsigned char)((KIND_GROUP0 + g) | (full_hp ? KIND_FULL : 0)); }
MG_HD bool kind_is_agent(int t) { return t >= KIND_GROUP0 && t != KIND_FOOD; }
MG_HD int kind_group(int t) { return (t & KIND_GROUP_MASK) - KIND_GROUP0; }
enum : int { RANK_NONE = -1, DEATH_NEVER = 0x7fffffff, DEATH_BEFORE = -1 };
enum : unsigned { MVKEY_NONE = 0xffffffffu };

enum : unsigned char { FLAG_DEAD = 1, FLAG_ABSORBED = 2 };
enum : unsigned char { MV_NONE = 0, MV_OOB = 1, MV_STATIC_FAIL = 2, MV_PENDING_FAIL = 3, MV_OK = 4, MV_ABSORBED = 5, MV_SKIPPED = 6 };

enum EventOp : unsigned char { OP_AND = 0, OP_OR, OP_NOT, OP_KILL, OP_AT, OP_IN, OP_COLLIDE, OP_ATTACK,
                               OP_DIE, OP_IN_A_LINE, OP_ALIGN, OP_NULL };

MG_HD int code_make(int g, int i) { return (g << 24) | i; }
MG_HD int code_group(int c) { return c >> 24; }
MG_HD int code_index(int c) { return c & 0xffffff; }

enum { DIR_EAST = 0, DIR_SOUTH = 1, DIR_WEST = 2, DIR_NORTH = 3 };

struct AgentSoA {
    int *x, *y;
    float *hp;
    int *act;
    int *id;
    float *next_reward, *last_reward;
    int *op_obj;
    unsigned char *last_op;
    unsigned char *flags;
    unsigned char *dir;
};

struct GroupDev {
    int body_w, body_l;
    float max_hp, damage, step_recover, kill_supply;
    float eat_ability, food_supply;
    float step_reward, kill_reward, dead_penalty, attack_penalty;
    int attack_in_group;
    int can_absorb;
    int view_w, view_h, view_x1, view_y1;
    int view_count;
    int view_xoff, view_yoff;
    int att_xoff, att_yoff;
    int n_move, attack_base, n_action, n_attack;
    int channel;
    int feature_size;
    const int *move_dx, *move_dy;
    const int *att_dx, *att_dy;
    const unsigned char *view_mask;
    int cap;
    int foff;
    AgentSoA soa[2];
    int *ev_rank;
};

struct ArenaHdr {
    uint32_t rng;
    uint32_t rng_next;
    int done;
    int n_attack;
    int any_dead;
    int changed[3];
    unsigned char rule_trig[MG_MAX_RULES];
    float grp_reward[MG_MAX_GROUPS];
    int n_cull[MG_MAX_GROUPS];
    int allq_viol[MG_MAX_ALLQ], allq_min[MG_MAX_ALLQ], allq_max[MG_MAX_ALLQ];
};

enum { ROLE_GROUP = 254, ROLE_ALL = 255 };
enum { IN_ANY = 0, IN_ALL = 1, IN_FIXED = 2 };
enum { RULE_GENERAL = 0, RULE_ONE_ANY = 1, RULE_DEAD = 2 };
enum { MG_HOT_RULES = 16, MG_HOT_PROG = 4, MG_HOT_RECV = 2 };

struct RuleInstr {
    unsigned char op;
    unsigned char role_a;
    unsigned char role_b;
    unsigned char allq;
    int i0, i1, i2, i3;
    int all_group;
};

struct RuleRecv { int role; int group; float value; };

struct RuleInput {
    int kind;
    int group, index;
    int has_obj, obj_group, obj_index;
};

struct RuleDev {
    int n_in; RuleInput in[MG_MAX_IN];
    int n_any; int any_in[MG_MAX_IN];
    int dead;
    int n_prog; RuleInstr prog[MG_MAX_PROG];
    int n_recv; RuleRecv recv[MG_MAX_RECV];
    int is_terminal;
};

struct RuleHot {
    unsigned char shape;
    unsigned char terminal;
    unsigned char group;
    unsigned char has_obj;
    int obj_group, obj_index;
    int simple_op;
};
struct RuleSmall {
    int n_prog, n_recv;
    RuleInstr prog[MG_HOT_PROG];
    RuleRecv recv[MG_HOT_RECV];
};

struct EngineDev {
    int A, W, H, G;
    int nsep, bandwidth, large_map;
    int minimap_mode, embedding_size, n_channel, channel_base;
    int food_mode;
    float *food;
    int turn_mode;
    int cap_total, max_body;
    int any_absorb;
    int scratch_stride;
    uint32_t pow2[32];
    GroupDev grp[MG_MAX_GROUPS];
    ArenaHdr *hdr;
    int *n, *dead_ct;
    int *off;
    int *done;
    int *occ, *claim_head;
    unsigned char *kind;
    float *hpn;
    int kpad, kw;
    long kplane;
    int *att_rank, *tgt, *in_head, *in_next, *death, *mv_nx, *mv_ny;
    unsigned *mv_key;
    float *hp_fin;
    unsigned char *mv_state;
    int *jv, *sh_head, *sh_next, *sh_first, *att_agent;
    int *cl_next;
    int n_rules; const RuleDev *rules;
    RuleSmall rule_small[MG_HOT_RULES];
    RuleHot rule_hot[MG_MAX_RULES];
    int n_allq;
    long long *counters;
    int *team_scratch;
    int *mm_count;
    int *mm_total;
};

struct StepArgs {
    unsigned curmask;
    int record_events;
    int n_order;
    int order[MG_MAX_GROUPS];
};

struct ObsArgs {
    unsigned curmask;
    int group;
    void *view;
    void *feature;
    int half;
};

enum InfoKind { INFO_ID = 0, INFO_POS, INFO_ALIVE, INFO_REWARD, INFO_ACTION_SCATTER, INFO_HP };

}
```

magent_b200/csrc/engine.cc:

```cpp
#include "engine.h"
#include "step_phases.h"

#include <math.h>
#include <stdarg.h>
#include <stdio.h>
#include <stdlib.h>
#include <string.h>
#include <algorithm>
#include <chrono>
#include <fstream>
#include <set>
#include <sstream>

#include "backend.h"
#include "host_expand.h"

namespace mg {

static std::string g_last_error;
const char *last_error() { return g_last_error.c_str(); }
void set_last_error(const std::string &s) { g_last_error = s; }

void fatal(const char *fmt, ...) {
    char buf[1024];
    va_list ap;
    va_start(ap, fmt);
    vsnprintf(buf, sizeof buf, fmt, ap);
    va_end(ap);
    g_last_error = buf;
    fprintf(stderr, "[magent_b200 FATAL] %s\n", buf);
    fflush(stderr);
    abort();
}

static bool strequ(const char *a, const char *b) { return strcmp(a, b) == 0; }

RangeTab make_circle_range(float radius, float inner_radius, int parity) {
    const double eps = 1e-8;
    RangeTab r;
    r.width = 2 * int(radius + eps) + parity;
    int center = (int)(radius);
    if (r.width % 2 != parity) r.width++;
    r.height = r.width;
    r.mask.assign((size_t)r.width * r.width, 0);
    double delta = (parity == 0 ? 0.5 : 0);
    for (int i = 0; i < r.width; i++) {
        for (int j = 0; j < r.width; j++) {
            double dis_x = fabs(j - center + delta);
            double dis_y = fabs(i - center + delta);
            double dis = sqrt(dis_x * dis_x + dis_y * dis_y);
            if (dis < radius + eps && dis > inner_radius - eps) {
                r.mask[(size_t)i * r.width + j] = 1;
                r.dx.push_back(j - center);
                r.dy.push_back(i - center);
                r.count++;
            }
        }
    }
    r.x1 = r.y1 = -center;
    r.x2 = r.y2 = r.width - center - 1;
    return r;
}

RangeTab make_sector_range(float angle, float radius, int parity) {
    static const double kPi = 3.1415926536;
    const double eps = 0.00001;
    RangeTab r;
    r.height = (int)(radius + 0.5);
    r.width = (int)(2 * radius * sin(angle / 2 * (kPi / 180)) + 0.5);
    if (r.width % 2 != parity) r.width--;
    if (r.width < 0) r.width = 0;
    r.mask.assign((size_t)r.width * r.height, 0);
    const double lim = tan(angle / 2 * kPi / 180) + eps;
    for (int i = 0; i < r.height; i++)
        for (int j = 0; j < r.width; j++) {
            const double dis_x = fabs(j - (r.width - 1) / 2.0), dis_y = fabs((double)(r.height - i));
            const double dis = sqrt(dis_x * dis_x + dis_y * dis_y);
            if (dis < radius + 0.2 + eps && dis_x / dis_y < lim) {
                r.mask[(size_t)i * r.width + j] = 1;
                r.dx.push_back(j - r.width / 2);
                r.dy.push_back(i - r.height);
                r.count++;
            }
        }
    r.x1 = -(r.width / 2); r.y1 = -r.height;
    r.x2 = (r.width - 1) / 2; r.y2 = -1;
    return r;
}

void HostGroup::clear() { resize(0); dead_ct = 0; n_cull = 0; }
void HostGroup::resize(int n) {
    x.resize(n); y.resize(n); id.resize(n); act.resize(n); op_obj.resize(n);
    hp.resize(n); next_reward.resize(n); last_reward.resize(n);
    last_op.resize(n); flags.resize(n); dir.resize(n);
}

Engine::Engine() {
    memset(&hE_, 0, sizeof hE_);
    arenas_.resize(1);
    arenas_[0].rng = minstd_seed(0);
}

Engine::~Engine() {
    free_device();
    if (h_feat_stage_) be::host_free(h_feat_stage_);
    if (bx_) be::destroy(bx_);
}

void Engine::check_group(int g, const char *where) const {
    if (g < 0 || g >= G()) fatal("invalid group handle %d in %s", g, where);
}

int Engine::group2channel(int g) const {
    int base = 1, scale = 2;
    if (food_mode_) base++;
    if (minimap_mode_) scale++;
    return base + g * scale;
}

int Engine::feature_size(int g) const {
    int f = embedding_size_ + group_type_[g]->n_action + 1;
    if (goal_mode_) f += 2;
    if (minimap_mode_) f += 2;
    return f;
}

void Engine::set_config(const char *key, void *p_value) {
    int ivalue = *(int *)p_value;
    bool bvalue = *(bool *)p_value;
    if (strequ(key, "map_width")) W_ = ivalue;
    else if (strequ(key, "map_height")) H_ = ivalue;
    else if (strequ(key, "food_mode")) {
        food_mode_ = bvalue;
    } else if (strequ(key, "turn_mode")) {
        turn_mode_ = bvalue;
    } else if (strequ(key, "minimap_mode")) minimap_mode_ = bvalue;
    else if (strequ(key, "goal_mode")) goal_mode_ = bvalue;
    else if (strequ(key, "embedding_size")) embedding_size_ = ivalue;
    else if (strequ(key, "render_dir")) render_dir_ = (const char *)p_value;
    else if (strequ(key, "seed")) {
        if (where_ == DEVICE) to_host(false);
        for (int a = 0; a < A_; ++a)
            if (sel_arena_ < 0 || sel_arena_ == a)
                arenas_[a].rng = minstd_seed((long long)ivalue + (sel_arena_ < 0 ? a : 0));
    }
    else if (strequ(key, "num_arenas")) {
        if (was_reset_) fatal("num_arenas must be configured before the first reset");
        if (ivalue < 1) fatal("num_arenas must be >= 1");
        A_ = ivalue;
        uint32_t seed0 = arenas_[0].rng;
        arenas_.assign(A_, HostArena());
        for (int a = 0; a < A_; ++a) arenas_[a].rng = a == 0 ? seed0 : minstd_seed(a);
    } else if (strequ(key, "device_id")) device_id_ = ivalue;
    else if (strequ(key, "host_path")) host_path_ = ivalue;
    else fatal("invalid argument in GridWorld::set_config : %s", key);
}

void Engine::register_agent_type(const char *name, int n, const char **keys, float *values) {
    std::string str(name);
    if (types_.count(str)) fatal("duplicated name of agent type in GridWorld::register_agent_type : %s", name);
    AgentTypeDef t;
    t.name = str;
    for (int i = 0; i < n; i++) {
        const char *k = keys[i];
        float v = values[i];
#define MG_SET_INT(f) if (strequ(k, #f)) { t.f = (int)(v + 0.5); continue; }
#define MG_SET_FLT(f) if (strequ(k, #f)) { t.f = v; continue; }
#define MG_SET_BOOL(f) if (strequ(k, #f)) { t.f = bool(int(v + 0.5)); continue; }
        MG_SET_INT(width) MG_SET_INT(length)
        MG_SET_FLT(speed) MG_SET_FLT(hp)
        MG_SET_FLT(view_radius) MG_SET_FLT(view_angle) MG_SET_FLT(attack_radius) MG_SET_FLT(attack_angle)
        MG_SET_FLT(hear_radius) MG_SET_FLT(speak_radius) MG_SET_INT(speak_ability)
        MG_SET_FLT(damage) MG_SET_FLT(trace) MG_SET_FLT(eat_ability)
        MG_SET_FLT(step_recover) MG_SET_FLT(kill_supply) MG_SET_FLT(food_supply)
        MG_SET_BOOL(attack_in_group) MG_SET_BOOL(can_absorb)
        MG_SET_FLT(step_reward) MG_SET_FLT(kill_reward) MG_SET_FLT(dead_penalty) MG_SET_FLT(attack_penalty)
#undef MG_SET_INT
#undef MG_SET_FLT
#undef MG_SET_BOOL
        if (strequ(k, "view_x_offset") || strequ(k, "view_y_offset") || strequ(k, "att_x_offset") ||
            strequ(k, "att_y_offset") || strequ(k, "turn_x_offset") || strequ(k, "turn_y_offset")) continue;
        fatal("invalid agent config in AgentType::AgentType : %s", k);
    }
    if (t.width < 1 || t.length < 1 || t.width * t.length > 16) fatal("unsupported body size %dx%d", t.width, t.length);

    int parity = t.width % 2;
    if (t.view_angle >= 180) {
        if (fabs(t.view_angle - 360) > 1e-5) fatal("only supports ranges with angle = 360, when angle > 180.");
        t.view = make_circle_range(t.view_radius, 0, parity);
    } else {
        t.view = make_sector_range(t.view_angle, t.view_radius, parity);
        if (t.view.width < 1 || t.view.height < 1) fatal("empty view range (view_radius %g, view_angle %g)", t.view_radius, t.view_angle);
    }
    if (t.attack_angle >= 180) {
        if (fabs(t.attack_angle - 360) > 1e-5) fatal("only supports ranges with angle = 360, when angle > 180.");
        t.attack = make_circle_range(t.attack_radius, t.width / 2.0f, parity);
    } else {
        t.attack = make_sector_range(t.attack_angle, t.attack_radius, parity);
    }
    t.move = make_circle_range(t.speed, 0, 1);
    t.view_x_offset = t.width / 2; t.view_y_offset = t.length / 2;
    t.att_x_offset = t.width / 2;  t.att_y_offset = t.length / 2;
    t.move_base = 0;
    t.turn_base = t.move.count;
    t.attack_base = t.turn_base + (turn_mode_ ? 2 : 0);
    t.n_action = t.attack_base + t.attack.count;
    types_.insert(std::make_pair(str, t));
}

void Engine::new_group(const char *type_name, int *handle) {
    auto it = types_.find(std::string(type_name));
    if (it == types_.end()) fatal("invalid name of agent type in new_group : %s", type_name);
    if (G() >= MG_MAX_GROUPS) fatal("too many groups (max %d)", (int)MG_MAX_GROUPS);
    if (where_ == DEVICE) to_host(false);
    *handle = G();
    group_type_.push_back(&it->second);
    for (auto &ar : arenas_) ar.groups.resize(G());
    refresh_host_counts();
}

void Engine::define_agent_symbol(int no, int group, int index) {
    if (no >= (int)symbols_.size()) symbols_.resize(no + 1);
    symbols_[no].group = group;
    symbols_[no].index = index;
}

void Engine::define_event_node(int no, int op, int *inputs, int n_inputs) {
    if (no >= (int)nodes_.size()) nodes_.resize(no + 1);
    nodes_[no].op = op;
    for (int i = 0; i < n_inputs; i++) nodes_[no].raw.push_back(inputs[i]);
}

void Engine::add_reward_rule(int on, int *receivers, float *values, int n_receiver,
                             bool is_terminal, bool auto_value) {
    RuleDef r;
    r.on = on;
    for (int i = 0; i < n_receiver; i++) { r.recv.push_back(receivers[i]); r.values.push_back(values[i]); }
    r.is_terminal = is_terminal;
    r.auto_value = auto_value;
    rules_.push_back(r);
}

namespace {
struct NodeInfo { std::set<int> related; std::map<int, int> infer; };

void collect(const std::vector<NodeDef> &nodes, int no, std::vector<NodeInfo> &info, std::vector<char> &seen) {
    if (seen[no]) return;
    seen[no] = 1;
    const NodeDef &n = nodes[no];
    NodeInfo &me = info[no];
    switch (n.op) {
        case OP_AND: case OP_OR:
            for (int q = 0; q < 2; ++q) {
                collect(nodes, n.raw[q], info, seen);
                me.related.insert(info[n.raw[q]].related.begin(), info[n.raw[q]].related.end());
                me.infer.insert(info[n.raw[q]].infer.begin(), info[n.raw[q]].infer.end());
            }
            break;
        case OP_NOT:
            collect(nodes, n.raw[0], info, seen);
            me.related = info[n.raw[0]].related;
            me.infer = info[n.raw[0]].infer;
            break;
        case OP_KILL: case OP_COLLIDE: case OP_ATTACK:
            me.related.insert(n.raw[0]); me.related.insert(n.raw[1]);
            me.infer.insert(std::make_pair(n.raw[0], n.raw[1]));
            break;
        case OP_AT: case OP_IN: case OP_DIE: case OP_IN_A_LINE: case OP_ALIGN:
            me.related.insert(n.raw[0]);
            break;
        default:
            fatal("invalid event op in GridWorld::collect_related_symbol");
    }
}
}

void Engine::compile_rules() {
    compiled_rules_.clear();
    n_allq_ = 0;
    if (rules_.size() > MG_MAX_RULES) fatal("too many reward rules (max %d)", (int)MG_MAX_RULES);
    std::vector<NodeInfo> info(nodes_.size());
    std::vector<char> seen(nodes_.size(), 0);
    for (size_t i = 0; i < nodes_.size(); ++i) collect(nodes_, (int)i, info, seen);

    for (size_t ri = 0; ri < rules_.size(); ++ri) {
        const RuleDef &rd = rules_[ri];
        const NodeInfo &on = info[rd.on];
        std::vector<int> input, infer;
        std::set<int> added;
        for (int s : on.related) {
            if (added.count(s)) continue;
            auto it = on.infer.find(s);
            if (it != on.infer.end()) {
                input.push_back(s); infer.push_back(it->second);
                added.insert(s); added.insert(it->second);
            }
        }
        for (int s : on.related)
            if (!added.count(s)) { input.push_back(s); infer.push_back(-1); }

        if (input.empty()) fatal("reward rule %d: the trigger event binds no agent symbol", (int)ri);
        if (input.size() > MG_MAX_IN)
            fatal("reward rule %d: %d input symbols (max %d)", (int)ri, (int)input.size(), (int)MG_MAX_IN);
        RuleDev R;
        memset(&R, 0, sizeof R);
        R.n_in = (int)input.size();
        std::map<int, int> writes;
        for (int k = 0; k < R.n_in; ++k) {
            const SymbolDef &sd = symbols_[input[k]];
            RuleInput &in = R.in[k];
            check_group(sd.group, "reward rule subject");
            in.group = sd.group; in.index = sd.index;
            in.kind = sd.index == -1 ? IN_ANY : sd.index == -2 ? IN_ALL : IN_FIXED;
            if (sd.index < -2) fatal("reward rule %d: invalid agent symbol index %d", (int)ri, sd.index);
            if (in.kind == IN_ANY) R.any_in[R.n_any++] = k;
            if (in.kind != IN_ALL) writes[input[k]] = 2 * k;
            in.has_obj = infer[k] >= 0;
            if (in.has_obj) {
                const SymbolDef &od = symbols_[infer[k]];
                check_group(od.group, "reward rule object");
                if (od.index == -2) fatal("reward rule %d: the object of attack/kill/collide cannot be a group", (int)ri);
                in.obj_group = od.group; in.obj_index = od.index;
                writes[infer[k]] = 2 * k + 1;
            } else if (in.kind == IN_FIXED) {
                R.dead = 1;
            }
        }
        auto role_of = [&](int sym) -> int {
            auto it = writes.find(sym);
            if (it == writes.end()) fatal("reward rule %d: symbol %d is not bound by the trigger event", (int)ri, sym);
            return it->second;
        };
        struct Lower {
            const std::vector<NodeDef> &nodes; const std::vector<SymbolDef> &syms; RuleDev &R;
            decltype(role_of) &role; int &n_allq; int ri;
            void subject(RuleInstr &I, int sym) {
                if (syms[sym].index == -2) {
                    if (n_allq >= MG_MAX_ALLQ) fatal("too many group-quantified ('all') events in the reward rules");
                    I.role_a = ROLE_ALL; I.all_group = syms[sym].group; I.allq = (unsigned char)n_allq++;
                } else {
                    I.role_a = (unsigned char)role(sym);
                }
            }
            void go(int no) {
                const NodeDef &n = nodes[no];
                RuleInstr I; memset(&I, 0, sizeof I);
                I.op = (unsigned char)n.op;
                switch (n.op) {
                    case OP_AND: case OP_OR: go(n.raw[0]); go(n.raw[1]); break;
                    case OP_NOT: go(n.raw[0]); break;
                    case OP_KILL: case OP_COLLIDE: case OP_ATTACK:
                        if (syms[n.raw[1]].index == -2)
                            fatal("reward rule %d: the object of attack/kill/collide cannot be a group", ri);
                        subject(I, n.raw[0]); I.role_b = (unsigned char)role(n.raw[1]); break;
                    case OP_AT: subject(I, n.raw[0]); I.i0 = n.raw[1]; I.i1 = n.raw[2]; break;
                    case OP_IN: subject(I, n.raw[0]);
                        I.i0 = n.raw[1]; I.i1 = n.raw[2]; I.i2 = n.raw[3]; I.i3 = n.raw[4]; break;
                    case OP_DIE: subject(I, n.raw[0]); break;
                    case OP_IN_A_LINE:
                        if (syms[n.raw[0]].index != -2) fatal("reward rule %d: 'in_a_line' needs an 'all' subject", ri);
                        subject(I, n.raw[0]); break;
                    case OP_ALIGN:
                        fatal("reward rule %d: 'align' reads GridWorld::counter_x/counter_y, which the reference never "
                              "allocates (GridWorld.cc:31, RewardEngine.cc:241-260: null dereference); not supported", ri);
                    default: fatal("invalid op of EventNode (%d)", n.op);
                }
                if (R.n_prog >= MG_MAX_PROG) fatal("reward rule trigger too large");
                R.prog[R.n_prog++] = I;
            }
        } lower{nodes_, symbols_, R, role_of, n_allq_, (int)ri};
        lower.go(rd.on);
        if (rd.recv.size() > MG_MAX_RECV) fatal("too many receivers in a reward rule");
        for (size_t q = 0; q < rd.recv.size(); ++q) {
            RuleRecv rc;
            const SymbolDef &sd = symbols_[rd.recv[q]];
            check_group(sd.group, "reward rule receiver");
            if (sd.index == -2) { rc.role = ROLE_GROUP; rc.group = sd.group; }
            else { rc.role = R.dead ? 0 : role_of(rd.recv[q]); rc.group = sd.group; }
            rc.value = rd.values[q];
            R.recv[R.n_recv++] = rc;
        }
        R.is_terminal = rd.is_terminal;
        compiled_rules_.push_back(R);
    }
    rules_compiled_ = true;
}

void Engine::refresh_host_counts() {
    h_off_.assign((size_t)G() * (A_ + 1), 0);
    for (int g = 0; g < G(); ++g)
        for (int a = 0; a < A_; ++a)
            h_off_[(size_t)g * (A_ + 1) + a + 1] = h_off_[(size_t)g * (A_ + 1) + a] +
                (g < (int)arenas_[a].groups.size() ? arenas_[a].groups[g].size() : 0);
}

void Engine::reset() {
    if (W_ <= 2 || H_ <= 2) fatal("map size not configured");
    settle_counts();
    if (where_ == DEVICE) {
        std::vector<ArenaHdr> hdr(A_);
        be::d2h(bx_, hdr.data(), hE_.hdr, sizeof(ArenaHdr) * A_);
        for (int a = 0; a < A_; ++a) {
            arenas_[a].rng = hdr[a].rng;
            for (int g = 0; g < (int)arenas_[a].groups.size(); ++g) arenas_[a].groups[g].grp_reward = hdr[a].grp_reward[g];
        }
        where_ = HOST;
    }
    file_ct_++; frame_ct_ = 0;
    large_map_ = (long)W_ * H_ > 99 * 99;
    nsep_ = large_map_ ? ((long)W_ * H_ > 1000 * 1000 ? 16 : 8) : 1;
    for (auto &ar : arenas_) {
        ar.id_counter = 0;
        ar.done = 0;
        ar.occ.assign((size_t)W_ * H_, OCC_EMPTY);
        ar.food.assign(food_mode_ ? (size_t)W_ * H_ : 0, 0.0f);
        for (int i = 0; i < W_; i++) { ar.occ[i] = OCC_WALL; ar.occ[(size_t)(H_ - 1) * W_ + i] = OCC_WALL; }
        for (int i = 0; i < H_; i++) { ar.occ[(size_t)i * W_] = OCC_WALL; ar.occ[(size_t)i * W_ + W_ - 1] = OCC_WALL; }
        ar.groups.resize(G());
        for (auto &g : ar.groups) g.clear();
    }
    if (!rules_compiled_) compile_rules();
    was_reset_ = true;
    order_.clear();
    refresh_host_counts();
}

bool Engine::host_is_blank(const HostArena &ar, int x, int y, int w, int h) const {
    if (x < 0 || y < 0 || x + w >= W_ || y + h >= H_) return false;
    for (int i = 0; i < w; i++)
        for (int j = 0; j < h; j++)
            if (ar.occ[(size_t)(y + j) * W_ + x + i] != OCC_EMPTY) return false;
    return true;
}

static inline uint32_t rng_next(uint32_t &state) { state = mulmod31(state, MINSTD_A); return state; }

void Engine::host_random_blank(HostArena &ar, int w, int h, int &x, int &y) {
    int tries = 0;
    for (;;) {
        x = (int)rng_next(ar.rng) % (W_ - w);
        y = (int)rng_next(ar.rng) % (H_ - h);
        if (host_is_blank(ar, x, y, w, h)) return;
        if (tries++ > W_ * H_) fatal("cannot find a blank position in a filled map");
    }
}

int Engine::host_add_wall(HostArena &ar, int x, int y) {
    if (x < 0 || y < 0 || x >= W_ || y >= H_) return 1;
    int &c = ar.occ[(size_t)y * W_ + x];
    if (c >= 0 || c == OCC_FOOD) return 1;
    c = OCC_WALL;
    return 0;
}

int Engine::host_add_agent(HostArena &ar, int g, int x, int y, int dir) {
    const AgentTypeDef &t = *group_type_[g];
    const bool upright = dir == DIR_NORTH || dir == DIR_SOUTH;
    const int bw = upright ? t.width : t.length, bh = upright ? t.length : t.width;
    if (!host_is_blank(ar, x, y, bw, bh)) return 1;
    HostGroup &hg = ar.groups[g];
    int i = hg.size();
    if (i >= (1 << 23)) fatal("too many agents in one group of one arena (max %d)", 1 << 23);
    hg.resize(i + 1);
    hg.x[i] = x; hg.y[i] = y; hg.id[i] = ar.id_counter++;
    hg.act[i] = t.n_action;
    hg.op_obj[i] = -1;
    hg.hp[i] = t.hp;
    hg.next_reward[i] = t.step_reward; hg.last_reward[i] = 0.0f;
    hg.last_op[i] = OP_NULL; hg.flags[i] = 0; hg.dir[i] = (unsigned char)dir;
    int code = code_make(g, i);
    for (int bx = 0; bx < bw; bx++)
        for (int by = 0; by < bh; by++)
            ar.occ[(size_t)(y + by) * W_ + x + bx] = code;
    return 0;
}

void Engine::add_agents(int group, int n, const char *method,
                        const int *pos_x, const int *pos_y, const int *pos_dir) {
    if (!was_reset_) fatal("add_agents before reset");
    if (where_ == DEVICE) to_host(false);
    const bool is_random = strequ(method, "random"), is_custom = strequ(method, "custom"),
               is_fill = strequ(method, "fill");
    if (!is_random && !is_custom && !is_fill) fatal("unsupported method in GridWorld::add_agents : %s", method);
    if (group != -1) check_group(group, "GridWorld::add_agents");
    for (int a = 0; a < A_; ++a) {
        if (sel_arena_ >= 0 && sel_arena_ != a) continue;
        HostArena &ar = arenas_[a];
        if (group == -1) {
            if (is_random) {
                for (int i = 0; i < n; i++) { int x, y; host_random_blank(ar, 1, 1, x, y); host_add_wall(ar, x, y); }
            } else if (is_custom) {
                for (int i = 0; i < n; i++) host_add_wall(ar, pos_x[i], pos_y[i]);
            } else {
                int x0 = pos_x[0], y0 = pos_x[1], x1 = x0 + pos_x[2], y1 = y0 + pos_x[3];
                for (int x = x0; x < x1; x++) for (int y = y0; y < y1; y++) host_add_wall(ar, x, y);
            }
        } else {
            const AgentTypeDef &t = *group_type_[group];
            if (is_random) {
                for (int i = 0; i < n; i++) {
                    const int dir = turn_mode_ ? (int)(rng_next(ar.rng) % 4u) : DIR_NORTH;
                    const bool upright = dir == DIR_NORTH || dir == DIR_SOUTH;
                    int x, y;
                    host_random_blank(ar, upright ? t.width : t.length, upright ? t.length : t.width, x, y);
                    host_add_agent(ar, group, x, y, dir);
                }
            } else if (is_custom) {
                for (int i = 0; i < n; i++) {
                    if (pos_dir && pos_dir[i] >= 4) fatal("invalid direction in GridWorld::add_agent");
                    host_add_agent(ar, group, pos_x[i], pos_y[i], turn_mode_ && pos_dir ? pos_dir[i] : DIR_NORTH);
                }
            } else {
                int x0 = pos_x[0], y0 = pos_x[1], x1 = x0 + pos_x[2], y1 = y0 + pos_x[3];
                const int dir = turn_mode_ ? pos_x[4] : DIR_NORTH;
                if (dir < 0 || dir >= 4) fatal("invalid direction in GridWorld::add_agent");
                const bool upright = dir == DIR_NORTH || dir == DIR_SOUTH;
                const int mw = upright ? t.width : t.length, mh = upright ? t.length : t.width;
                for (int x = x0; x < x1; x += mw)
                    for (int y = y0; y < y1; y += mh) host_add_agent(ar, group, x, y, dir);
            }
        }
    }
    refresh_host_counts();
}

void Engine::ensure_backend() {
    if (bx_) {
        if (device_id_ >= 0 && device_id_ != be::device_of(bx_)) fatal("device_id changed after the engine had started on device %d", be::device_of(bx_));
        return;
    }
    std::string err;
    bx_ = be::create(device_id_, &err);
    if (!bx_) fatal("no usable CUDA device for the B200 engine: %s (there is no CPU fallback)", err.c_str());
}

void *Engine::dalloc(size_t bytes) {
    void *p = be::dmalloc(bx_, bytes ? bytes : 16);
    dev_allocs_.push_back(p);
    return p;
}

void Engine::free_device() {
    for (void *p : dev_allocs_) be::dfree(bx_, p);
    dev_allocs_.clear();
    if (d_view_stage_) be::dfree(bx_, d_view_stage_);
    if (d_feat_stage_) be::dfree(bx_, d_feat_stage_);
    if (d_io_stage_) be::dfree(bx_, d_io_stage_);
    d_view_stage_ = d_feat_stage_ = nullptr; d_io_stage_ = nullptr;
    view_stage_bytes_ = feat_stage_bytes_ = io_stage_bytes_ = 0;
    dE_ = nullptr;
    cap_.clear();
}

void *Engine::io_stage(size_t bytes) {
    if (bytes > io_stage_bytes_) {
        if (d_io_stage_) be::dfree(bx_, d_io_stage_);
        io_stage_bytes_ = bytes + bytes / 4 + 256;
        d_io_stage_ = be::dmalloc(bx_, io_stage_bytes_);
    }
    return d_io_stage_;
}

int Engine::max_agents_per_arena() const {
    int m = 0;
    for (int a = 0; a < A_; ++a) {
        int s = 0;
        for (int g = 0; g < G(); ++g) s += count(g, a);
        m = std::max(m, s);
    }
    return m;
}

template <class T>
static T *upload_vec(be::Ctx *bx_, std::vector<void *> &allocs, const std::vector<T> &v) {
    T *p = (T *)be::dmalloc(bx_, std::max<size_t>(v.size(), 1) * sizeof(T));
    allocs.push_back(p);
    if (!v.empty()) be::h2d(bx_, p, v.data(), v.size() * sizeof(T));
    return p;
}

void Engine::to_device() {
    if (where_ == DEVICE) return;
    if (!was_reset_) fatal("environment used before reset");
    ensure_backend();
    const int Gn = G();
    std::vector<int> need(Gn, 0);
    for (int g = 0; g < Gn; ++g) {
        for (int a = 0; a < A_; ++a) need[g] = std::max(need[g], count(g, a));
        need[g] = std::max(64, (need[g] + 63) / 64 * 64);
    }
    int pad = 0;
    for (int g = 0; g < Gn; ++g) {
        const AgentTypeDef &t = *group_type_[g];
        const int ox = t.view_x_offset + t.view.x1, oy = t.view_y_offset + t.view.y1;
        const int ext[4] = {-ox, ox + t.view.width - 1, -oy, oy + t.view.height - 1};
        for (int e : ext) pad = std::max(pad, e + (turn_mode_ ? std::max(t.width, t.length) : 0));
    }
    bool realloc = dE_ == nullptr || hE_.A != A_ || hE_.W != W_ || hE_.H != H_ || hE_.G != Gn || hE_.kpad != pad ||
                   (hE_.food != nullptr) != food_mode_;
    if (!realloc) for (int g = 0; g < Gn; ++g) if (need[g] > cap_[g]) realloc = true;
    if (realloc) {
        std::vector<long long> saved_counters;
        if (dE_ != nullptr) { saved_counters.resize(MG_N_COUNTERS); be::d2h(bx_, saved_counters.data(), hE_.counters, sizeof(long long) * MG_N_COUNTERS); }
        free_device();
        memset(&hE_, 0, sizeof hE_);
        cap_ = need;
        hE_.A = A_; hE_.W = W_; hE_.H = H_; hE_.G = Gn;
        int foff = 0, max_body = 1, max_cells = 1;
        for (int g = 0; g < Gn; ++g) {
            const AgentTypeDef &t = *group_type_[g];
            GroupDev &D = hE_.grp[g];
            D.body_w = t.width; D.body_l = t.length;
            D.max_hp = t.hp; D.damage = t.damage; D.step_recover = t.step_recover; D.kill_supply = t.kill_supply;
            D.eat_ability = t.eat_ability; D.food_supply = t.food_supply;
            D.step_reward = t.step_reward; D.kill_reward = t.kill_reward;
            D.dead_penalty = t.dead_penalty; D.attack_penalty = t.attack_penalty;
            D.attack_in_group = t.attack_in_group;
            D.can_absorb = t.can_absorb;
            if (t.can_absorb) hE_.any_absorb = 1;
            D.view_w = t.view.width; D.view_h = t.view.height; D.view_x1 = t.view.x1; D.view_y1 = t.view.y1;
            D.view_count = t.view.count;
            D.view_xoff = t.view_x_offset; D.view_yoff = t.view_y_offset;
            D.att_xoff = t.att_x_offset; D.att_yoff = t.att_y_offset;
            D.n_move = t.move.count; D.attack_base = t.attack_base; D.n_action = t.n_action; D.n_attack = t.attack.count;
            D.channel = group2channel(g);
            D.feature_size = feature_size(g);
            D.move_dx = upload_vec(bx_, dev_allocs_, t.move.dx); D.move_dy = upload_vec(bx_, dev_allocs_, t.move.dy);
            D.att_dx = upload_vec(bx_, dev_allocs_, t.attack.dx); D.att_dy = upload_vec(bx_, dev_allocs_, t.attack.dy);
            D.view_mask = upload_vec(bx_, dev_allocs_, t.view.mask);
            D.cap = cap_[g];
            D.foff = foff; foff += cap_[g];
            max_body = std::max(max_body, t.width * t.length);
            max_cells = std::max(max_cells, t.view.width * t.view.height);
            size_t n = (size_t)A_ * cap_[g];
            for (int b = 0; b < 2; ++b) {
                AgentSoA &s = D.soa[b];
                s.x = (int *)dalloc(n * 4); s.y = (int *)dalloc(n * 4); s.hp = (float *)dalloc(n * 4);
                s.act = (int *)dalloc(n * 4); s.id = (int *)dalloc(n * 4);
                s.next_reward = (float *)dalloc(n * 4); s.last_reward = (float *)dalloc(n * 4);
                s.op_obj = (int *)dalloc(n * 4);
                s.last_op = (unsigned char *)dalloc(n); s.flags = (unsigned char *)dalloc(n); s.dir = (unsigned char *)dalloc(n);
            }
            D.ev_rank = (int *)dalloc(n * 4);
        }
        hE_.cap_total = foff; hE_.max_body = max_body; hE_.scratch_stride = foff;
        size_t cells = (size_t)A_ * W_ * H_, sc = (size_t)A_ * foff;
        hE_.hdr = (ArenaHdr *)dalloc(sizeof(ArenaHdr) * A_);
        hE_.n = (int *)dalloc((size_t)Gn * A_ * 4); hE_.dead_ct = (int *)dalloc((size_t)Gn * A_ * 4);
        hE_.off = (int *)dalloc((size_t)Gn * (A_ + 1) * 4);
        hE_.done = (int *)dalloc((size_t)A_ * 4);
        hE_.occ = (int *)dalloc(cells * 4); hE_.claim_head = (int *)dalloc(cells * 4);
        hE_.food = food_mode_ ? (float *)dalloc(cells * 4) : nullptr;
        {
            hE_.kpad = pad; hE_.kw = W_ + 2 * pad; hE_.kplane = (long)hE_.kw * (H_ + 2 * pad);
            hE_.kind = (unsigned char *)dalloc((size_t)A_ * hE_.kplane + 16);
            hE_.hpn = (float *)dalloc(((size_t)A_ * hE_.kplane + 4) * 4);
            be::dmemset(bx_, hE_.hpn, 0, ((size_t)A_ * hE_.kplane + 4) * 4);
        }
        hE_.att_rank = (int *)dalloc(sc * 4); hE_.tgt = (int *)dalloc(sc * 4);
        hE_.in_head = (int *)dalloc(sc * 4); hE_.in_next = (int *)dalloc(sc * 4);
        hE_.death = (int *)dalloc(sc * 4); hE_.mv_nx = (int *)dalloc(sc * 4); hE_.mv_ny = (int *)dalloc(sc * 4);
        hE_.mv_key = (unsigned *)dalloc(sc * 4); hE_.hp_fin = (float *)dalloc(sc * 4);
        hE_.mv_state = (unsigned char *)dalloc(sc);
        hE_.jv = (int *)dalloc(sc * 4); hE_.sh_head = (int *)dalloc(sc * 4); hE_.sh_next = (int *)dalloc(sc * 4);
        hE_.sh_first = (int *)dalloc(sc * 4); hE_.att_agent = (int *)dalloc(sc * 4);
        hE_.cl_next = (int *)dalloc(sc * max_body * 4);
        hE_.counters = (long long *)dalloc(sizeof(long long) * MG_N_COUNTERS);
        if (saved_counters.empty()) be::dmemset(bx_, hE_.counters, 0, sizeof(long long) * MG_N_COUNTERS);
        else be::h2d(bx_, hE_.counters, saved_counters.data(), sizeof(long long) * MG_N_COUNTERS);
        hE_.team_scratch = (int *)dalloc(sizeof(int) * 2 * 4096);
        hE_.mm_count = (int *)dalloc((size_t)A_ * Gn * max_cells * 4);
        hE_.mm_total = (int *)dalloc((size_t)A_ * Gn * 4);
        d_mm_val_ = (float *)dalloc((size_t)A_ * Gn * max_cells * 4);
        hE_.rules = (const RuleDev *)dalloc(sizeof(RuleDev) * (compiled_rules_.size() + 1));
        dE_ = (EngineDev *)dalloc(sizeof(EngineDev));
    }
    hE_.nsep = nsep_; hE_.large_map = large_map_; hE_.bandwidth = (W_ + nsep_ - 1) / nsep_;
    hE_.minimap_mode = minimap_mode_; hE_.embedding_size = embedding_size_; hE_.turn_mode = turn_mode_ ? 1 : 0;
    hE_.food_mode = food_mode_ ? 1 : 0;
    hE_.n_channel = n_channel(); hE_.channel_base = group2channel(0);
    {
        uint32_t p = MINSTD_A;
        for (int b = 0; b < 32; ++b) { hE_.pow2[b] = p; p = mulmod31(p, p); }
    }
    hE_.n_rules = (int)compiled_rules_.size();
    if (hE_.n_rules) be::h2d(bx_, (void *)hE_.rules, compiled_rules_.data(), sizeof(RuleDev) * compiled_rules_.size());
    hE_.n_allq = n_allq_;
    for (int r = 0; r < hE_.n_rules; ++r) {
        const RuleDev &R = compiled_rules_[r];
        RuleHot &H = hE_.rule_hot[r];
        H.shape = R.dead ? RULE_DEAD : (R.n_in == 1 && R.n_any == 1) ? RULE_ONE_ANY : RULE_GENERAL;
        H.terminal = R.is_terminal ? 1 : 0;
        H.group = (unsigned char)R.in[0].group; H.has_obj = (unsigned char)R.in[0].has_obj;
        H.obj_group = R.in[0].obj_group; H.obj_index = R.in[0].obj_index;
        H.simple_op = 0;
        if (H.shape == RULE_ONE_ANY && R.in[0].has_obj && R.n_prog == 1 && R.prog[0].role_a == 0 && R.prog[0].role_b == 1 &&
            (R.prog[0].op == OP_KILL || R.prog[0].op == OP_ATTACK || R.prog[0].op == OP_COLLIDE))
            H.simple_op = R.prog[0].op;
        if (r < MG_HOT_RULES) {
            RuleSmall &Sm = hE_.rule_small[r];
            memset(&Sm, 0, sizeof Sm);
            Sm.n_prog = -1;
            if (R.n_prog <= MG_HOT_PROG && R.n_recv <= MG_HOT_RECV) {
                Sm.n_prog = R.n_prog; Sm.n_recv = R.n_recv;
                for (int q = 0; q < R.n_prog; ++q) Sm.prog[q] = R.prog[q];
                for (int q = 0; q < R.n_recv; ++q) Sm.recv[q] = R.recv[q];
            }
        }
    }
    for (int g = 0; g < Gn; ++g) hE_.grp[g].feature_size = feature_size(g);
    curmask_ = 0;

    std::vector<int> ibuf; std::vector<float> fbuf; std::vector<unsigned char> bbuf;
    for (int g = 0; g < Gn; ++g) {
        const size_t cap = cap_[g], n = (size_t)A_ * cap;
        const AgentSoA &s = hE_.grp[g].soa[0];
        auto up_i = [&](int *dst, std::vector<int> HostGroup::*m) {
            ibuf.assign(n, 0);
            for (int a = 0; a < A_; ++a) { const auto &v = arenas_[a].groups[g].*m; std::copy(v.begin(), v.end(), ibuf.begin() + a * cap); }
            be::h2d(bx_, dst, ibuf.data(), n * 4);
        };
        auto up_f = [&](float *dst, std::vector<float> HostGroup::*m) {
            fbuf.assign(n, 0);
            for (int a = 0; a < A_; ++a) { const auto &v = arenas_[a].groups[g].*m; std::copy(v.begin(), v.end(), fbuf.begin() + a * cap); }
            be::h2d(bx_, dst, fbuf.data(), n * 4);
        };
        auto up_b = [&](unsigned char *dst, std::vector<unsigned char> HostGroup::*m) {
            bbuf.assign(n, 0);
            for (int a = 0; a < A_; ++a) { const auto &v = arenas_[a].groups[g].*m; std::copy(v.begin(), v.end(), bbuf.begin() + a * cap); }
            be::h2d(bx_, dst, bbuf.data(), n);
        };
        up_i(s.x, &HostGroup::x); up_i(s.y, &HostGroup::y); up_i(s.act, &HostGroup::act);
        up_i(s.id, &HostGroup::id); up_i(s.op_obj, &HostGroup::op_obj);
        up_f(s.hp, &HostGroup::hp); up_f(s.next_reward, &HostGroup::next_reward); up_f(s.last_reward, &HostGroup::last_reward);
        up_b(s.last_op, &HostGroup::last_op); up_b(s.flags, &HostGroup::flags); up_b(s.dir, &HostGroup::dir);
    }
    for (int a = 0; a < A_; ++a)
        be::h2d(bx_, hE_.occ + (size_t)a * W_ * H_, arenas_[a].occ.data(), (size_t)W_ * H_ * 4);
    if (food_mode_)
        for (int a = 0; a < A_; ++a) {
            arenas_[a].food.resize((size_t)W_ * H_, 0.0f);
            be::h2d(bx_, hE_.food + (size_t)a * W_ * H_, arenas_[a].food.data(), (size_t)W_ * H_ * 4);
        }
    {
        std::vector<unsigned char> kp((size_t)hE_.kplane);
        for (int a = 0; a < A_; ++a) {
            std::fill(kp.begin(), kp.end(), (unsigned char)0);
            const std::vector<int> &occ = arenas_[a].occ;
            for (int y = 0; y < H_; ++y)
                for (int x = 0; x < W_; ++x) {
                    const int o = occ[(size_t)y * W_ + x];
                    kp[(size_t)(y + hE_.kpad) * hE_.kw + x + hE_.kpad] =
                        o == OCC_WALL ? KIND_WALL : o == OCC_FOOD ? KIND_FOOD : o >= 0 ?
                        kind_agent(code_group(o), arenas_[a].groups[code_group(o)].hp[code_index(o)] == group_type_[code_group(o)]->hp) : KIND_EMPTY;
                }
            be::h2d(bx_, hE_.kind + (size_t)a * hE_.kplane, kp.data(), kp.size());
        }
        std::vector<float> hp((size_t)hE_.kplane);
        for (int a = 0; a < A_; ++a) {
            std::fill(hp.begin(), hp.end(), 0.0f);
            for (int g = 0; g < Gn; ++g) {
                const HostGroup &hg = arenas_[a].groups[g];
                const AgentTypeDef &t = *group_type_[g];
                for (int i = 0; i < hg.size(); ++i) {
                    if (hg.flags[i] & FLAG_DEAD) continue;
                    const bool upright = !turn_mode_ || hg.dir[i] == DIR_NORTH || hg.dir[i] == DIR_SOUTH;
                    const int bw = upright ? t.width : t.length, bh = upright ? t.length : t.width;
                    const float v = hg.hp[i] / t.hp;
                    for (int bx = 0; bx < bw; ++bx)
                        for (int by = 0; by < bh; ++by)
                            hp[(size_t)(hg.y[i] + by + hE_.kpad) * hE_.kw + hg.x[i] + bx + hE_.kpad] = v;
                }
            }
            be::h2d(bx_, hE_.hpn + (size_t)a * hE_.kplane, hp.data(), hp.size() * 4);
        }
    }
    be::dmemset(bx_, hE_.claim_head, 0xff, (size_t)A_ * W_ * H_ * 4);
    {
        std::vector<ArenaHdr> hdr(A_);
        std::vector<int> n((size_t)Gn * A_), dc((size_t)Gn * A_), done(A_);
        for (int a = 0; a < A_; ++a) {
            memset(&hdr[a], 0, sizeof(ArenaHdr));
            hdr[a].rng = hdr[a].rng_next = arenas_[a].rng;
            hdr[a].done = done[a] = arenas_[a].done;
            for (int g = 0; g < Gn; ++g) {
                hdr[a].grp_reward[g] = arenas_[a].groups[g].grp_reward;
                hdr[a].n_cull[g] = arenas_[a].groups[g].n_cull;
                n[(size_t)g * A_ + a] = arenas_[a].groups[g].size();
                dc[(size_t)g * A_ + a] = arenas_[a].groups[g].dead_ct;
            }
        }
        be::h2d(bx_, hE_.hdr, hdr.data(), sizeof(ArenaHdr) * A_);
        be::h2d(bx_, hE_.n, n.data(), n.size() * 4);
        be::h2d(bx_, hE_.dead_ct, dc.data(), dc.size() * 4);
        be::h2d(bx_, hE_.done, done.data(), done.size() * 4);
        be::h2d(bx_, hE_.off, h_off_.data(), h_off_.size() * 4);
    }
    be::h2d(bx_, dE_, &hE_, sizeof(EngineDev));
    ++state_version_;
    may_have_dead_ = true;
    where_ = DEVICE;
}

void Engine::to_host(bool keep_device_authoritative) {
    if (where_ == HOST) return;
    settle_counts();
    const int Gn = G();
    std::vector<int> ibuf; std::vector<float> fbuf; std::vector<unsigned char> bbuf;
    std::vector<int> dc((size_t)Gn * A_);
    be::d2h(bx_, dc.data(), hE_.dead_ct, dc.size() * 4);
    std::vector<ArenaHdr> hdr(A_);
    be::d2h(bx_, hdr.data(), hE_.hdr, sizeof(ArenaHdr) * A_);
    for (int g = 0; g < Gn; ++g) {
        const size_t cap = cap_[g], n = (size_t)A_ * cap;
        const AgentSoA &s = hE_.grp[g].soa[(curmask_ >> g) & 1u];
        for (int a = 0; a < A_; ++a) arenas_[a].groups[g].resize(count(g, a));
        auto dn_i = [&](const int *src, std::vector<int> HostGroup::*m) {
            ibuf.resize(n); be::d2h(bx_, ibuf.data(), src, n * 4);
            for (int a = 0; a < A_; ++a) { auto &v = arenas_[a].groups[g].*m; std::copy(ibuf.begin() + a * cap, ibuf.begin() + a * cap + v.size(), v.begin()); }
        };
        auto dn_f = [&](const float *src, std::vector<float> HostGroup::*m) {
            fbuf.resize(n); be::d2h(bx_, fbuf.data(), src, n * 4);
            for (int a = 0; a < A_; ++a) { auto &v = arenas_[a].groups[g].*m; std::copy(fbuf.begin() + a * cap, fbuf.begin() + a * cap + v.size(), v.begin()); }
        };
        auto dn_b = [&](const unsigned char *src, std::vector<unsigned char> HostGroup::*m) {
            bbuf.resize(n); be::d2h(bx_, bbuf.data(), src, n);
            for (int a = 0; a < A_; ++a) { auto &v = arenas_[a].groups[g].*m; std::copy(bbuf.begin() + a * cap, bbuf.begin() + a * cap + v.size(), v.begin()); }
        };
        dn_i(s.x, &HostGroup::x); dn_i(s.y, &HostGroup::y); dn_i(s.act, &HostGroup::act);
        dn_i(s.id, &HostGroup::id); dn_i(s.op_obj, &HostGroup::op_obj);
        dn_f(s.hp, &HostGroup::hp); dn_f(s.next_reward, &HostGroup::next_reward); dn_f(s.last_reward, &HostGroup::last_reward);
        dn_b(s.last_op, &HostGroup::last_op); dn_b(s.flags, &HostGroup::flags); dn_b(s.dir, &HostGroup::dir);
        for (int a = 0; a < A_; ++a) {
            arenas_[a].groups[g].dead_ct = dc[(size_t)g * A_ + a];
            arenas_[a].groups[g].grp_reward = hdr[a].grp_reward[g];
            arenas_[a].groups[g].n_cull = hdr[a].n_cull[g];
        }
    }
    for (int a = 0; a < A_; ++a) {
        arenas_[a].occ.resize((size_t)W_ * H_);
        be::d2h(bx_, arenas_[a].occ.data(), hE_.occ + (size_t)a * W_ * H_, (size_t)W_ * H_ * 4);
        if (food_mode_) {
            arenas_[a].food.resize((size_t)W_ * H_);
            be::d2h(bx_, arenas_[a].food.data(), hE_.food + (size_t)a * W_ * H_, (size_t)W_ * H_ * 4);
        }
        arenas_[a].rng = hdr[a].rng;
        arenas_[a].done = hdr[a].done;
    }
    if (!keep_device_authoritative) where_ = HOST;
}

void Engine::stage_reserve(void *&p, size_t &have, size_t need) {
    if (need <= have) return;
    if (p) be::dfree(bx_, p);
    have = need + need / 8 + 256;
    p = be::dmalloc(bx_, have);
}

void Engine::get_observation(int group, void **bufs, int half) {
    check_group(group, "GridWorld::get_observation");
    to_device();
    if (!(be::is_device_ptr(bufs[0]) && be::is_device_ptr(bufs[1]))) settle_counts();
    const int n = total(group);
    if (n == 0) return;
    const AgentTypeDef &t = *group_type_[group];
    const size_t esz = half ? 2 : 4;
    const size_t vbytes = (size_t)n * t.view.height * t.view.width * n_channel() * esz;
    const size_t fbytes = (size_t)n * feature_size(group) * esz;
    const bool vdev = be::is_device_ptr(bufs[0]), fdev = be::is_device_ptr(bufs[1]);
    if (prep_version_ != state_version_ || prep_vw_ != t.view.width || prep_vh_ != t.view.height ||
        prep_skip_absorbed_ != t.can_absorb) {
        be::launch_obs_prepare(bx_, dE_, hE_, curmask_, group, minimap_mode_ ? d_mm_val_ : nullptr);
        prep_version_ = state_version_; prep_vw_ = t.view.width; prep_vh_ = t.view.height; prep_skip_absorbed_ = t.can_absorb;
    }
    if (host_path_ < 0) {
        const char *e = getenv("MAGENT_B200_HOST_PATH");
        host_path_ = (e && !strcmp(e, "dense")) ? 0 : (e && !strcmp(e, "wire")) ? 2 : 1;
    }
    if (!vdev && !fdev && !half && (host_path_ == 2 || (host_path_ == 1 && vbytes >= ((size_t)16 << 20))) && t.view.height * t.view.width < 0xffff &&
        (long long)t.view.height * t.view.width * n_channel() < (1ll << 30)) {
        get_observation_wire(group, bufs);
        return;
    }
    ObsArgs O;
    O.curmask = curmask_; O.group = group; O.half = half ? 1 : 0;
    if (vdev) O.view = bufs[0];
    else { stage_reserve(d_view_stage_, view_stage_bytes_, vbytes); O.view = d_view_stage_; }
    if (fdev) O.feature = bufs[1];
    else { stage_reserve(d_feat_stage_, feat_stage_bytes_, fbytes); O.feature = d_feat_stage_; }
    be::launch_obs(bx_, dE_, hE_, O, minimap_mode_ ? d_mm_val_ : nullptr, n);
    if (!vdev) { be::d2h(bx_, bufs[0], d_view_stage_, vbytes); io_[IO_D2H] += (long long)vbytes; }
    if (!fdev) { be::d2h(bx_, bufs[1], d_feat_stage_, fbytes); io_[IO_D2H] += (long long)fbytes; }
}

void Engine::get_observation_wire(int group, void **bufs) {
    const int n = total(group);
    const AgentTypeDef &t = *group_type_[group];
    const size_t fbytes = (size_t)n * feature_size(group) * 4;
    ObsArgs O;
    O.curmask = curmask_; O.group = group; O.half = 0;
    O.view = nullptr;
    stage_reserve(d_feat_stage_, feat_stage_bytes_, fbytes);
    O.feature = d_feat_stage_;
    const auto t0 = std::chrono::steady_clock::now();
    be::WireDesc W;
    be::obs_wire_begin(bx_, dE_, hE_, O, minimap_mode_ ? d_mm_val_ : nullptr, n, &W);
    const auto t1 = std::chrono::steady_clock::now();
    const bool fpinned = be::is_pinned_host_ptr(bufs[1]);
    if (!fpinned && fbytes > h_feat_stage_bytes_) {
        if (h_feat_stage_) be::host_free(h_feat_stage_);
        h_feat_stage_bytes_ = fbytes + fbytes / 8 + 256;
        h_feat_stage_ = be::host_alloc(h_feat_stage_bytes_);
        if (!h_feat_stage_) fatal("cannot allocate %zu bytes of page-locked staging", h_feat_stage_bytes_);
    }
    be::dma_d2h_async(bx_, fpinned ? bufs[1] : h_feat_stage_, d_feat_stage_, fbytes);
    ExpandGeom g;
    memset(&g, 0, sizeof g);
    g.C = n_channel(); g.cells = t.view.height * t.view.width; g.rec = g.cells * g.C; g.G = G();
    g.minimap = minimap_mode_ ? 1 : 0;
    const int stride = 2 + (minimap_mode_ ? 1 : 0);
    for (int j = 0; j < G(); ++j) {
        int rel = j - group; if (rel < 0) rel += G();
        g.mm_ch[j] = group2channel(0) + rel * stride + 2;
    }
    be::Ctx *bx = bx_;
    expand_views(g, W, (float *)bufs[0], [bx](int w) { be::obs_wire_wait(bx, w); });
    const auto t2 = std::chrono::steady_clock::now();
    be::dma_wait(bx_, 0);
    if (!fpinned) parallel_copy(bufs[1], h_feat_stage_, fbytes);
    const auto t3 = std::chrono::steady_clock::now();
    io_[IO_US_WIRE] += std::chrono::duration_cast<std::chrono::microseconds>(t1 - t0).count();
    io_[IO_US_EXPAND] += std::chrono::duration_cast<std::chrono::microseconds>(t2 - t1).count();
    io_[IO_US_FEATURE] += std::chrono::duration_cast<std::chrono::microseconds>(t3 - t2).count();
    io_[IO_D2H] += (long long)W.n_total * (long long)sizeof(be::WireHdr) + W.chunk_base[W.n_chunks] * (long long)sizeof(be::WireMark) +
                   (long long)(W.n_chunks + 1) * 8 + (W.mm ? (long long)A_ * W.mm_stride * 4 : 0) + (long long)fbytes;
    io_[IO_HOST_WRITTEN] += (long long)n * g.rec * 4 + (fpinned ? 0 : (long long)fbytes);
}

void Engine::set_action(int group, const int *actions) {
    check_group(group, "GridWorld::set_action");
    to_device();
    if (!be::is_device_ptr(actions)) settle_counts();
    const int n = total(group);
    if (std::find(order_.begin(), order_.end(), group) == order_.end()) order_.push_back(group);
    if (n == 0) return;
    const void *src = actions;
    if (!be::is_device_ptr(actions)) {
        void *st = io_stage((size_t)n * 4);
        be::h2d(bx_, st, actions, (size_t)n * 4);
        io_[IO_H2D] += (long long)n * 4;
        src = st;
    }
    be::launch_info(bx_, dE_, hE_, curmask_, INFO_ACTION_SCATTER, group, const_cast<void *>(src), n);
}

void Engine::random_actions(int group, unsigned long long seed) {
    check_group(group, "random_actions");
    to_device();
    if (std::find(order_.begin(), order_.end(), group) == order_.end()) order_.push_back(group);
    const int n = total(group);
    if (n == 0) return;
    be::launch_random_actions(bx_, dE_, hE_, curmask_, group, seed * 0x9E3779B97F4A7C15ull + (++rand_calls_), n);
}

void Engine::step(int *done) {
    to_device();
    StepArgs S;
    memset(&S, 0, sizeof S);
    S.curmask = curmask_;
    S.record_events = first_render_ ? 0 : 1;
    S.n_order = (int)order_.size();
    for (int k = 0; k < S.n_order; ++k) S.order[k] = order_[k];
    be::launch_step(bx_, dE_, hE_, S, max_agents_per_arena());
    ++state_version_;
    order_.clear();
    if (be::is_device_ptr(done)) {
        be::launch_done_to_device(bx_, dE_, hE_, done);
        may_have_dead_ = true;
        done_stale_ = true;
        if (!first_render_) collect_attack_events();
        return;
    }
    std::vector<int> d(A_);
    be::read_done(bx_, hE_, d.data());
    io_[IO_D2H] += (long long)A_ * 4;
    done_stale_ = false;
    int all = 1;
    for (int a = 0; a < A_; ++a) { arenas_[a].done = d[a] & 1; all &= arenas_[a].done; may_have_dead_ |= (d[a] & 2) != 0; }
    *done = all;
    if (!first_render_) collect_attack_events();
}

void Engine::get_reward(int group, float *buf) {
    check_group(group, "GridWorld::get_reward");
    to_device();
    if (!be::is_device_ptr(buf)) settle_counts();
    const int n = total(group);
    if (n == 0) return;
    if (be::is_device_ptr(buf)) { be::launch_info(bx_, dE_, hE_, curmask_, INFO_REWARD, group, buf, n); return; }
    void *st = io_stage((size_t)n * 4);
    be::launch_info(bx_, dE_, hE_, curmask_, INFO_REWARD, group, st, n);
    be::d2h(bx_, buf, st, (size_t)n * 4);
    io_[IO_D2H] += (long long)n * 4;
}

void Engine::clear_dead() {
    to_device();
    settle_counts();
    be::launch_cull(bx_, dE_, hE_, curmask_, max_agents_per_arena());
    ++state_version_;
    curmask_ ^= (1u << G()) - 1u;
    if (!may_have_dead_) return;
    may_have_dead_ = false;
    be::launch_offsets(bx_, dE_, hE_);
    if (be::capturing(bx_)) { ++capture_culls_; counts_unknown_ = true; return; }
    be::counts_fetch_begin(bx_, hE_.off, h_off_.size());
    counts_pending_ = true;
}

void Engine::settle_counts() {
    if (counts_unknown_ && !be::capturing(bx_)) {
        counts_unknown_ = false;
        counts_pending_ = false;
        be::d2h(bx_, h_off_.data(), hE_.off, h_off_.size() * 4);
        io_[IO_D2H] += (long long)h_off_.size() * 4;
        return;
    }
    if (!counts_pending_) return;
    memcpy(h_off_.data(), be::counts_fetch_wait(bx_), h_off_.size() * sizeof(int));
    io_[IO_D2H] += (long long)h_off_.size() * 4;
    counts_pending_ = false;
}

void Engine::set_goal(int group, const char *method, const int *) {
    check_group(group, "GridWorld::set_goal");
    if (!strequ(method, "random")) fatal("invalid goal type in GridWorld::set_goal");
    if (!was_reset_) fatal("set_goal before reset");
    if (where_ == DEVICE) to_host(false);
    for (int a = 0; a < A_; ++a) {
        if (sel_arena_ >= 0 && sel_arena_ != a) continue;
        HostArena &ar = arenas_[a];
        for (int i = 0, n = ar.groups[group].size(); i < n; ++i) { rng_next(ar.rng); rng_next(ar.rng); }
    }
}

void Engine::collect_attack_events() {
    settle_counts();
    const int a = sel_arena_ >= 0 ? sel_arena_ : 0;
    struct Ev { int rank, id, x, y; };
    std::vector<Ev> evs;
    for (int g = 0; g < G(); ++g) {
        const int n = count(g, a);
        if (n == 0) continue;
        const AgentTypeDef &t = *group_type_[g];
        const AgentSoA &s = hE_.grp[g].soa[(curmask_ >> g) & 1u];
        const size_t base = (size_t)a * cap_[g];
        std::vector<int> rank(n), x(n), y(n), act(n), id(n);
        be::d2h(bx_, rank.data(), hE_.grp[g].ev_rank + base, (size_t)n * 4);
        be::d2h(bx_, x.data(), s.x + base, (size_t)n * 4); be::d2h(bx_, y.data(), s.y + base, (size_t)n * 4);
        be::d2h(bx_, act.data(), s.act + base, (size_t)n * 4); be::d2h(bx_, id.data(), s.id + base, (size_t)n * 4);
        std::vector<unsigned char> dir(n, (unsigned char)DIR_NORTH);
        if (turn_mode_) be::d2h(bx_, dir.data(), s.dir + base, (size_t)n);
        for (int i = 0; i < n; ++i) {
            if (rank[i] < 0) continue;
            const int k = act[i] - t.attack_base;
            int rx, ry, dx, dy;
            dir_real(hE_.grp[g], dir[i], rx, ry);
            dir_rot(dir[i], t.att_x_offset + t.attack.dx[k], t.att_y_offset + t.attack.dy[k], dx, dy);
            evs.push_back({rank[i], id[i], x[i] + rx + dx, y[i] + ry + dy});
        }
    }
    std::sort(evs.begin(), evs.end(), [](const Ev &p, const Ev &q) { return p.rank < q.rank; });
    attack_events_.clear();
    for (const Ev &e : evs) attack_events_.push_back({e.id, e.x, e.y});
}

void Engine::render_next_file() { file_ct_++; frame_ct_ = 0; }

namespace {
template <typename T> void print_json(std::ofstream &os, const char *key, T value, bool last = false) {
    os << "\"" << key << "\": " << value;
    if (last) os << std::endl; else os << "," << std::endl;
}
std::string rgba_string(int r, int g, int b, float alpha) {
    std::stringstream ss;
    ss << "\"rgba(" << r << "," << g << "," << b << "," << alpha << ")\"";
    return ss.str();
}
}

void Engine::render() {
    static const int colors[][3] = {{192, 64, 64}, {64, 64, 192}, {64, 192, 64}, {64, 64, 64}};
    if (render_dir_ == "___debug___") return;
    if (first_render_) {
        first_render_ = false;
        std::ofstream f(render_dir_ + "/" + "config.json");
        f << "{" << std::endl;
        print_json(f, "width", W_);
        print_json(f, "height", H_);
        print_json(f, "static-file", "\"static.map\"");
        print_json(f, "obstacle-style", rgba_string(127, 127, 127, 1));
        print_json(f, "dynamic-file-directory", "\".\"");
        print_json(f, "attack-style", rgba_string(63, 63, 63, 0.8));
        print_json(f, "minimap-width", 300);
        print_json(f, "minimap-height", 250);
        f << "\"group\" : [" << std::endl;
        for (int i = 0; i < G(); i++) {
            const AgentTypeDef &t = *group_type_[i];
            const int *c = colors[i % 4];
            f << "{" << std::endl;
            print_json(f, "height", t.length);
            print_json(f, "width", t.width);
            print_json(f, "style", rgba_string(c[0], c[1], c[2], 1));
            print_json(f, "anchor", "[0, 0]");
            print_json(f, "max-speed", (int)t.speed);
            print_json(f, "speed-style", rgba_string(c[0], c[1], c[2], 0.01));
            print_json(f, "vision-radius", t.view_radius);
            print_json(f, "vision-angle", t.view_angle);
            print_json(f, "vision-style", rgba_string(c[0], c[1], c[2], 0.2));
            print_json(f, "attack-radius", t.attack_radius);
            print_json(f, "attack-angle", t.attack_angle);
            print_json(f, "attack-style", rgba_string(c[0], c[1], c[2], 0.1));
            print_json(f, "broadcast-radius", 1, true);
            f << (i == G() - 1 ? "}" : "},") << std::endl;
        }
        f << "]" << std::endl << "}" << std::endl;
    }
    if (render_dir_.empty()) return;
    if (was_reset_ && where_ == DEVICE) to_host(true);
    const HostArena &ar = arenas_[sel_arena_ >= 0 ? sel_arena_ : 0];
    std::ofstream fout(render_dir_ + "/" + "video_" + std::to_string(file_ct_) + ".txt",
                       frame_ct_ == 0 ? std::ios::out : std::ios::app);
    if (frame_ct_ == 0) {
        std::vector<int> walls;
        for (int i = 0; i < W_ * H_; i++) if (ar.occ[i] == OCC_WALL) walls.push_back(i);
        fout << "W" << " " << walls.size() << std::endl;
        for (int w : walls) fout << w % W_ << " " << w / W_ << std::endl;
    }
    int num_agents = 0;
    for (int g = 0; g < G(); g++) {
        const HostGroup &hg = ar.groups[g];
        num_agents += hg.size();
        if (group_type_[g]->can_absorb)
            for (int j = 0; j < hg.size(); j++) if (!(hg.flags[j] & FLAG_ABSORBED)) num_agents--;
    }
    fout << "F" << " " << num_agents << " " << (int)attack_events_.size() << " " << 0 << std::endl;
    for (int g = 0; g < G(); g++) {
        const HostGroup &hg = ar.groups[g];
        const AgentTypeDef &t = *group_type_[g];
        for (int j = 0; j < hg.size(); j++) {
            if (t.can_absorb && !(hg.flags[j] & FLAG_ABSORBED)) continue;
            int hp = std::max(0, int(100 * hg.hp[j] / t.hp));
            hp = std::min(hp, 100);
            static const int dir2angle[] = {0, 90, 180, 270};
            fout << hg.id[j] << " " << hp << " " << dir2angle[hg.dir[j] & 3] << " " << hg.x[j] << " " << hg.y[j] << " " << g << std::endl;
        }
    }
    for (const AttackEvent &e : attack_events_) fout << 0 << " " << e.id << " " << e.x << " " << e.y << std::endl;
    if (frame_ct_++ > frame_per_file_) { frame_ct_ = 0; file_ct_++; }
}

void Engine::sync() { if (bx_) be::sync(bx_); }
void Engine::graph_begin() {
    to_device();
    settle_counts();
    if (!first_render_) fatal("graph capture while rendering is not supported");
    capture_mask_ = curmask_; capture_culls_ = 0;
    if (!be::capture_begin(bx_)) fatal("this backend has no CUDA graph support");
}
int Engine::graph_end() {
    const int id = be::capture_end(bx_);
    if (curmask_ != capture_mask_) fatal("a captured step sequence must contain an even number of clear_dead calls (got %d)", capture_culls_);
    return id;
}
void Engine::graph_launch(int id, int times) {
    to_device();
    for (int k = 0; k < times; ++k) be::graph_launch(bx_, id);
    if (times > 0) { ++state_version_; counts_unknown_ = true; counts_pending_ = false; may_have_dead_ = true; done_stale_ = true; }
}
void Engine::get_io_stats(long long *out, int cap) { for (int i = 0; i < cap && i < IO_N; ++i) out[i] = io_[i]; }
void *Engine::stream() { ensure_backend(); return be::stream_handle(bx_); }
void Engine::set_profiling(bool on) { ensure_backend(); be::profile_enable(bx_, on); }
void Engine::get_profile(double *ms, long long *n) { *ms = 0; *n = 0; if (bx_) be::profile_read(bx_, ms, n); }

int Engine::get_counters(long long *out, int cap) {
    int n = std::min<int>(cap, MG_N_COUNTERS);
    if (where_ != DEVICE && dE_ == nullptr) { for (int i = 0; i < n; ++i) out[i] = 0; return n; }
    std::vector<long long> c(MG_N_COUNTERS);
    be::d2h(bx_, c.data(), hE_.counters, sizeof(long long) * MG_N_COUNTERS);
    for (int i = 0; i < n; ++i) out[i] = c[i];
    return n;
}

void Engine::get_info(int group, const char *name, void *void_buffer) {
    settle_counts();
    int *ib = (int *)void_buffer;
    float *fb = (float *)void_buffer;
    if (strequ(name, "num")) {
        check_group(group, "get_info(num)");
        ib[0] = total(group);
    } else if (strequ(name, "id") || strequ(name, "pos") || strequ(name, "alive") || strequ(name, "hp")) {
        check_group(group, "get_info");
        to_device();
        const int n = total(group);
        if (n == 0) return;
        int kind = strequ(name, "id") ? INFO_ID : strequ(name, "pos") ? INFO_POS : strequ(name, "alive") ? INFO_ALIVE : INFO_HP;
        size_t bytes = kind == INFO_POS ? (size_t)n * 8 : kind == INFO_ALIVE ? (size_t)n : (size_t)n * 4;
        if (be::is_device_ptr(void_buffer)) { be::launch_info(bx_, dE_, hE_, curmask_, kind, group, void_buffer, n); return; }
        void *st = io_stage(bytes);
        be::launch_info(bx_, dE_, hE_, curmask_, kind, group, st, n);
        be::d2h(bx_, void_buffer, st, bytes);
    } else if (strequ(name, "arena_num")) {
        check_group(group, "get_info(arena_num)");
        for (int a = 0; a < A_; ++a) ib[a] = count(group, a);
    } else if (strequ(name, "arena_done")) {
        if (done_stale_ && where_ == DEVICE) {
            std::vector<int> d(A_);
            be::read_done(bx_, hE_, d.data());
            for (int a = 0; a < A_; ++a) arenas_[a].done = d[a] & 1;
            done_stale_ = false;
        }
        for (int a = 0; a < A_; ++a) ib[a] = arenas_[a].done;
    } else if (strequ(name, "action_space")) {
        check_group(group, "get_info"); ib[0] = group_type_[group]->n_action;
    } else if (strequ(name, "view_space")) {
        check_group(group, "get_info");
        ib[0] = group_type_[group]->view.height; ib[1] = group_type_[group]->view.width; ib[2] = n_channel();
    } else if (strequ(name, "feature_space")) {
        check_group(group, "get_info"); ib[0] = feature_size(group);
    } else if (strequ(name, "view2attack")) {
        check_group(group, "get_info");
        const AgentTypeDef &t = *group_type_[group];
        for (int i = 0; i < t.view.height * t.view.width; ++i) ib[i] = -1;
        const int cells = t.view.height * t.view.width;
        for (int i = 0; i < t.attack.count; ++i) {
            const long idx = (long)(t.attack.dy[i] - t.view.y1) * t.view.width + (t.attack.dx[i] - t.view.x1);
            if (idx >= 0 && idx < cells) ib[idx] = i;
        }
    } else if (strequ(name, "attack_base")) {
        check_group(group, "get_info"); ib[0] = group_type_[group]->attack_base;
    } else if (strequ(name, "both_attack")) {
        ib[0] = 0;
    } else if (strequ(name, "groups_info")) {
        static const int colors[][3] = {{192, 64, 64}, {64, 64, 192}, {64, 192, 64}, {64, 64, 64}};
        for (int i = 0; i < G(); i++) {
            ib[i * 5 + 0] = group_type_[i]->width; ib[i * 5 + 1] = group_type_[i]->length;
            for (int c = 0; c < 3; ++c) ib[i * 5 + 2 + c] = colors[i % 4][c];
        }
    } else if (strequ(name, "walls_info") || strequ(name, "global_minimap") || strequ(name, "mean_info") ||
               strequ(name, "render_window_info") || strequ(name, "attack_event")) {
        to_host(true);
        const HostArena &ar = arenas_[sel_arena_ >= 0 ? sel_arena_ : 0];
        if (strequ(name, "walls_info")) {
            int ct = 0;
            for (int i = 0; i < W_ * H_; i++)
                if (ar.occ[i] == OCC_WALL) { ++ct; ib[ct * 2] = i % W_; ib[ct * 2 + 1] = i / W_; }
            ib[0] = ct;
        } else if (strequ(name, "global_minimap")) {
            int vh = (int)lround(fb[0]), vw = (int)lround(fb[1]);
            int ng = G();
            for (int i = 0; i < vh * vw * ng; ++i) fb[i] = 0.0f;
            int scale_h = (H_ + vh - 1) / vh, scale_w = (W_ + vw - 1) / vw;
            for (int i = 0; i < ng; i++) {
                int ch = ((i - group) % ng + ng) % ng;
                const HostGroup &hg = ar.groups[i];
                for (int j = 0; j < hg.size(); j++) fb[((hg.y[j] / scale_h) * vw + hg.x[j] / scale_w) * ng + ch] += 1.0f;
                for (int j = 0; j < vh * vw; j++) fb[j * ng + ch] /= (float)hg.size();
            }
        } else if (strequ(name, "mean_info")) {
            check_group(group, "get_info(mean_info)");
            const HostGroup &hg = ar.groups[group];
            int na = group_type_[group]->n_action;
            float sx = 0, sy = 0;
            std::vector<int> ctr(na + 1, 0);
            for (int i = 0; i < hg.size(); i++) { sx += hg.x[i]; sy += hg.y[i]; if (hg.act[i] >= 0 && hg.act[i] <= na) ctr[hg.act[i]]++; }
            fb[0] = sx / hg.size(); fb[1] = sy / hg.size();
            for (int i = 0; i < na; i++) fb[2 + i] = (float)(1.0 * ctr[i] / hg.size());
        } else if (strequ(name, "render_window_info")) {
            first_render_ = false;
            int x1 = ib[0], y1 = ib[1], x2 = ib[2], y2 = ib[3], ct = 1;
            for (int g = 0; g < G(); g++) {
                const HostGroup &hg = ar.groups[g];
                for (int j = 0; j < hg.size(); j++) {
                    if (hg.x[j] < x1 || hg.x[j] > x2 || hg.y[j] < y1 || hg.y[j] > y2) continue;
                    if (group_type_[g]->can_absorb && !(hg.flags[j] & FLAG_ABSORBED)) continue;
                    ib[ct * 4] = hg.id[j]; ib[ct * 4 + 1] = hg.x[j]; ib[ct * 4 + 2] = hg.y[j]; ib[ct * 4 + 3] = g; ct++;
                }
            }
            ib[0] = ct - 1; ib[1] = (int)attack_events_.size();
        } else if (strequ(name, "attack_event")) {
            for (size_t i = 0; i < attack_events_.size(); i++) {
                ib[i * 3] = attack_events_[i].id; ib[i * 3 + 1] = attack_events_[i].x; ib[i * 3 + 2] = attack_events_[i].y;
            }
        }
    } else {
        fatal("unsupported info name in GridWorld::get_info : %s", name);
    }
}

}
```

Measured before the change: 874.1 million.

## Enable programmatic dependent launch and fold offsets/done reductions into last-CTA tails

Launches all stream kernels with programmatic stream serialization and adds griddepcontrol wait/trigger so each kernel's launch and prologue can overlap its predecessor. The separate offsets scan and done-reduce kernels are folded into the cull and step kernels, run by the last CTA to finish (a global atomic ticket), removing two launches per step. Profiling switches from CUDA event pairs, which would break PDL edges, to in-kernel globaltimer stamps. Risks include ordering subtleties because pdl_trigger is issued early, and serialized single-CTA tail work at the end of the step and cull kernels.

```diff
diff --git a/magent_b200/csrc/backend_cuda.cu b/magent_b200/csrc/backend_cuda.cu
--- a/magent_b200/csrc/backend_cuda.cu
+++ b/magent_b200/csrc/backend_cuda.cu
@@ -7,6 +7,7 @@
 #include <string.h>
 #include <atomic>
 #include <mutex>
+#include <utility>
 #include <vector>
 
 #include "backend.h"
@@ -42,14 +43,19 @@
     have = smem;
 }
 
+enum { TICKET_STEP = 0, TICKET_CULL = 1, TICKET_N = 2 };
+
 struct Ctx {
     int device = 0, sms = 0;
     cudaStream_t stream = nullptr;
     cudaStream_t copy = nullptr;
     cudaEvent_t ev_wire = nullptr, ev_done = nullptr;
+    unsigned *tickets = nullptr;
+    int *done_written = nullptr;
+    bool offsets_written = false;
     bool profile = false;
-    std::vector<cudaEvent_t> events;
-    size_t events_used = 0;
+    unsigned long long *prof_ts = nullptr;
+    size_t prof_cap = 0, prof_used = 0;
     float *mm_pad = nullptr; size_t mm_pad_n = 0; int mm_stride = 0;
     int4 *obs_hdr = nullptr; size_t obs_hdr_n = 0;
     struct ObsCfg { size_t smem = (size_t)-1; int ctas_per_sm = 1; } obs_cfg[8];
@@ -114,6 +120,8 @@
     CUDA_CHECK(cudaEventCreateWithFlags(&c->ev_wire, cudaEventDisableTiming));
     CUDA_CHECK(cudaEventCreateWithFlags(&c->ev_done, cudaEventDisableTiming));
     CUDA_CHECK(cudaEventCreateWithFlags(&c->ev_counts, cudaEventDisableTiming));
+    CUDA_CHECK(cudaMalloc((void **)&c->tickets, TICKET_N * sizeof(unsigned)));
+    CUDA_CHECK(cudaMemset(c->tickets, 0, TICKET_N * sizeof(unsigned)));
     return c;
 }
 void destroy(Ctx *c) {
@@ -121,7 +129,7 @@
     cudaSetDevice(c->device);
     for (cudaGraphExec_t e : c->graphs) if (e) cudaGraphExecDestroy(e);
     cudaStreamSynchronize(c->stream); cudaStreamSynchronize(c->copy);
-    for (cudaEvent_t e : c->events) cudaEventDestroy(e);
+    cudaFree(c->tickets); cudaFree(c->prof_ts);
     for (cudaEvent_t e : c->wave_events) cudaEventDestroy(e);
     for (cudaEvent_t e : c->dma_events) cudaEventDestroy(e);
     cudaEventDestroy(c->ev_wire); cudaEventDestroy(c->ev_done);
@@ -183,24 +191,42 @@
 }
 void sync(Ctx *c) { no_capture(c, "a synchronisation"); DeviceGuard g(c); CUDA_CHECK(cudaStreamSynchronize(c->stream)); CUDA_CHECK(cudaStreamSynchronize(c->copy)); }
 long long launch_count() { return g_launches.load(); }
-void profile_enable(Ctx *c, bool on) { c->profile = on; c->events_used = 0; }
-static void profile_pair(Ctx *c, cudaEvent_t *e0, cudaEvent_t *e1) {
-    if (c->events_used + 2 > c->events.size()) {
-        for (int i = 0; i < 64; ++i) { cudaEvent_t e; CUDA_CHECK(cudaEventCreate(&e)); c->events.push_back(e); }
-    }
-    *e0 = c->events[c->events_used]; *e1 = c->events[c->events_used + 1];
-    c->events_used += 2;
+static void profile_reset(Ctx *c, size_t lo, size_t hi) {
+    if (hi <= lo) return;
+    std::vector<unsigned long long> init(2 * (hi - lo));
+    for (size_t i = 0; i < hi - lo; ++i) { init[2 * i] = ~0ull; init[2 * i + 1] = 0ull; }
+    h2d(c, c->prof_ts + 2 * lo, init.data(), init.size() * sizeof(unsigned long long));
+}
+void profile_enable(Ctx *c, bool on) {
+    DeviceGuard g(c);
+    profile_reset(c, 0, c->prof_used);
+    c->profile = on; c->prof_used = 0;
+}
+static unsigned long long *profile_slot(Ctx *c) {
+    if (c->prof_used == c->prof_cap) {
+        const size_t cap = c->prof_cap ? 2 * c->prof_cap : 1024;
+        unsigned long long *p = nullptr;
+        CUDA_CHECK(cudaMalloc((void **)&p, cap * 2 * sizeof(unsigned long long)));
+        if (c->prof_ts) {
+            CUDA_CHECK(cudaMemcpyAsync(p, c->prof_ts, c->prof_cap * 2 * sizeof(unsigned long long), cudaMemcpyDeviceToDevice, c->stream));
+            CUDA_CHECK(cudaStreamSynchronize(c->stream));
+            cudaFree(c->prof_ts);
+        }
+        c->prof_ts = p;
+        const size_t old = c->prof_cap;
+        c->prof_cap = cap;
+        profile_reset(c, old, cap);
+    }
+    return c->prof_ts + 2 * c->prof_used++;
 }
 void profile_read(Ctx *c, double *ms, long long *n) {
     DeviceGuard g(c);
-    double total = 0.0;
-    for (size_t i = 0; i + 1 < c->events_used; i += 2) {
-        CUDA_CHECK(cudaEventSynchronize(c->events[i + 1]));
-        float t = 0;
-        CUDA_CHECK(cudaEventElapsedTime(&t, c->events[i], c->events[i + 1]));
-        total += t;
-    }
-    *ms = total; *n = (long long)(c->events_used / 2);
+    std::vector<unsigned long long> ts(2 * c->prof_used);
+    d2h(c, ts.data(), c->prof_ts, ts.size() * sizeof(unsigned long long));
+    double total_ns = 0.0;
+    for (size_t i = 0; i < c->prof_used; ++i)
+        if (ts[2 * i + 1] >= ts[2 * i]) total_ns += (double)(ts[2 * i + 1] - ts[2 * i]);
+    *ms = total_ns * 1e-6; *n = (long long)c->prof_used;
 }
 
 bool capture_begin(Ctx *c) {
@@ -237,6 +263,55 @@
     ++g_launches;
     cudaError_t e = cudaGetLastError();
     if (e != cudaSuccess) mg::fatal("kernel launch failed (%s): %s", what, cudaGetErrorString(e));
+}
+
+#ifndef MG_PDL
+#define MG_PDL 1
+#endif
+__device__ __forceinline__ void pdl_wait() {
+#if MG_PDL
+    asm volatile("griddepcontrol.wait;" ::: "memory");
+#endif
+}
+__device__ __forceinline__ void pdl_trigger() {
+#if MG_PDL
+    asm volatile("griddepcontrol.launch_dependents;" ::: "memory");
+#endif
+}
+
+__device__ __forceinline__ unsigned long long globaltimer_ns() {
+    unsigned long long t;
+    asm volatile("mov.u64 %0, %%globaltimer;" : "=l"(t));
+    return t;
+}
+
+template <typename... KArgs, typename... Args>
+static void launch_pdl(Ctx *c, const char *what, void (*kernel)(KArgs...), dim3 grid, dim3 block, size_t smem, Args &&...args) {
+    cudaLaunchAttribute attr[1];
+    attr[0].id = cudaLaunchAttributeProgrammaticStreamSerialization;
+    attr[0].val.programmaticStreamSerializationAllowed = 1;
+    cudaLaunchConfig_t cfg = {};
+    cfg.gridDim = grid;
+    cfg.blockDim = block;
+    cfg.dynamicSmemBytes = smem;
+    cfg.stream = c->stream;
+    cfg.attrs = attr;
+    cfg.numAttrs = MG_PDL ? 1 : 0;
+    CUDA_CHECK(cudaLaunchKernelEx(&cfg, kernel, std::forward<Args>(args)...));
+    post_launch(what);
+}
+
+__device__ __forceinline__ bool last_cta_ticket(unsigned *ticket) {
+    __shared__ bool last_s;
+    __threadfence();
+    __syncthreads();
+    if (threadIdx.x == 0) {
+        const bool last = atomicAdd(ticket, 1u) == gridDim.x - 1;
+        if (last) { *ticket = 0; __threadfence(); }
+        last_s = last;
+    }
+    __syncthreads();
+    return last_s;
 }
 
 __device__ __forceinline__ int block_excl_scan(int v, int &total) {
@@ -459,7 +534,37 @@
     sE->scratch_stride = 0;
 }
 
-__global__ void __launch_bounds__(STEP_THREADS) step_kernel_cta(const EngineDev *gE, StepArgs S, int scratch_in_smem) {
+__device__ __forceinline__ void reduce_done(const EngineDev &E, int *out) {
+    __shared__ int all_s;
+    if (threadIdx.x == 0) all_s = 1;
+    __syncthreads();
+    int all = 1;
+    for (int a = threadIdx.x; a < E.A; a += blockDim.x) all &= __ldcg(E.done + a) & 1;
+    if (!all) all_s = 0;
+    __syncthreads();
+    if (threadIdx.x == 0) *out = all_s;
+}
+
+__device__ __forceinline__ void group_offsets(const EngineDev &E) {
+    const int A = E.A;
+    for (int g = 0; g < E.G; ++g) {
+        const int *n = E.n + (size_t)g * A;
+        int *off = E.off + (size_t)g * (A + 1);
+        int running = 0;
+        for (int tile = 0; tile < A; tile += blockDim.x) {
+            int a = tile + threadIdx.x;
+            int v = a < A ? __ldcg(n + a) : 0;
+            int tot;
+            int ex = block_excl_scan(v, tot);
+            if (a < A) off[a] = running + ex;
+            running += tot;
+        }
+        if (threadIdx.x == 0) off[A] = running;
+    }
+}
+
+__global__ void __launch_bounds__(STEP_THREADS) step_kernel_cta(const EngineDev *gE, StepArgs S, int scratch_in_smem,
+                                                                unsigned *ticket) {
     extern __shared__ __align__(16) unsigned char step_smem[];
     __shared__ EngineDev sE;
     load_engine(&sE, gE);
@@ -467,6 +572,8 @@
         if (threadIdx.x == 0) step_scratch_to_smem(&sE, step_smem);
         __syncthreads();
     }
+    pdl_wait();
+    pdl_trigger();
     __shared__ int relax_flags[3];
     __shared__ int counter_sums[MG_N_COUNTERS];
     __shared__ GroupEnum enum_store[2];
@@ -477,6 +584,7 @@
     c.enum_smem = enum_store;
     for (int k = 0; k < MG_N_COUNTERS; ++k) c.cnt[k] = 0;
     for (int a = blockIdx.x; a < sE.A; a += gridDim.x) run_step(c, sE, S, a);
+    if (S.done_out && last_cta_ticket(ticket)) reduce_done(sE, S.done_out);
 }
 
 __global__ void __launch_bounds__(STEP_THREADS) step_kernel_grid(const EngineDev *gE, StepArgs S) {
@@ -491,14 +599,17 @@
     for (int a = 0; a < sE.A; ++a) run_step(c, sE, S, a);
 }
 
-__global__ void __launch_bounds__(STEP_THREADS) cull_kernel_cta(const EngineDev *gE, unsigned curmask) {
+__global__ void __launch_bounds__(STEP_THREADS) cull_kernel_cta(const EngineDev *gE, unsigned curmask, unsigned *ticket) {
     __shared__ EngineDev sE;
     load_engine(&sE, gE);
+    pdl_wait();
+    pdl_trigger();
     CtaCtx c;
     c.flag_smem = nullptr;
     c.cnt_smem = nullptr;
     c.enum_smem = nullptr;
     for (int a = blockIdx.x; a < sE.A; a += gridDim.x) run_cull(c, sE, curmask, a);
+    if (last_cta_ticket(ticket)) group_offsets(sE);
 }
 
 __global__ void __launch_bounds__(STEP_THREADS) cull_kernel_grid(const EngineDev *gE, unsigned curmask) {
@@ -527,6 +638,17 @@
     return g > 4096 ? 4096 : g;
 }
 
+__global__ void __launch_bounds__(1024) offsets_kernel(const EngineDev *gE) {
+    pdl_wait();
+    pdl_trigger();
+    group_offsets(*gE);
+}
+__global__ void __launch_bounds__(256) done_reduce_kernel(const EngineDev *gE, int *out) {
+    pdl_wait();
+    pdl_trigger();
+    reduce_done(*gE, out);
+}
+
 void launch_step(Ctx *c, const EngineDev *dE, const EngineDev &hE, const StepArgs &S, int max_agents) {
     DeviceGuard guard(c);
     const int g_sms = c->sms;
@@ -536,6 +658,7 @@
         void *args[] = {(void *)&dE, (void *)&s};
         CUDA_CHECK(cudaLaunchCooperativeKernel((const void *)step_kernel_grid, dim3(grid), dim3(GRID_THREADS), args, 0, c->stream));
         post_launch("step_kernel_grid");
+        c->done_written = nullptr;
     } else {
         const size_t sbytes = step_scratch_bytes(hE.cap_total, hE.max_body);
         static const int smem_pref = getenv("MAGENT_B200_STEP_SMEM") ? atoi(getenv("MAGENT_B200_STEP_SMEM")) : -1;
@@ -553,8 +676,8 @@
         CUDA_CHECK(cudaOccupancyMaxActiveBlocksPerMultiprocessor(&per_sm, step_kernel_cta, threads, smem));
         if (per_sm < 1) per_sm = 1;
         int grid = hE.A < per_sm * g_sms ? hE.A : per_sm * g_sms;
-        step_kernel_cta<<<grid, threads, smem, c->stream>>>(dE, S, in_smem ? 1 : 0);
-        post_launch("step_kernel_cta");
+        launch_pdl(c, "step_kernel_cta", step_kernel_cta, grid, threads, smem, dE, S, in_smem ? 1 : 0, c->tickets + TICKET_STEP);
+        c->done_written = S.done_out;
     }
 }
 
@@ -566,37 +689,21 @@
         void *args[] = {(void *)&dE, (void *)&curmask};
         CUDA_CHECK(cudaLaunchCooperativeKernel((const void *)cull_kernel_grid, dim3(grid), dim3(GRID_THREADS), args, 0, c->stream));
         post_launch("cull_kernel_grid");
+        c->offsets_written = false;
     } else {
         int grid = hE.A < 8 * g_sms ? hE.A : 8 * g_sms;
         static const int cull_pref = getenv("MAGENT_B200_CULL_THREADS") ? atoi(getenv("MAGENT_B200_CULL_THREADS")) : 0;
         int threads = max_agents >= 768 ? 512 : step_block_size(g_sms, hE.A, max_agents);
         if (cull_pref >= 32 && cull_pref <= STEP_THREADS) threads = cull_pref & ~31;
-        cull_kernel_cta<<<grid, threads, 0, c->stream>>>(dE, curmask);
-        post_launch("cull_kernel_cta");
-    }
-}
-
-__global__ void __launch_bounds__(1024) offsets_kernel(const EngineDev *gE) {
-    const int g = blockIdx.x;
-    const int A = gE->A;
-    const int *n = gE->n + (size_t)g * A;
-    int *off = gE->off + (size_t)g * (A + 1);
-    int running = 0;
-    for (int tile = 0; tile < A; tile += blockDim.x) {
-        int a = tile + threadIdx.x;
-        int v = a < A ? n[a] : 0;
-        int tot;
-        int ex = block_excl_scan(v, tot);
-        if (a < A) off[a] = running + ex;
-        running += tot;
-    }
-    if (threadIdx.x == 0) off[A] = running;
-}
-
-void launch_offsets(Ctx *c, const EngineDev *dE, const EngineDev &hE) {
-    DeviceGuard guard(c);
-    offsets_kernel<<<hE.G, 1024, 0, c->stream>>>(dE);
-    post_launch("offsets_kernel");
+        launch_pdl(c, "cull_kernel_cta", cull_kernel_cta, grid, threads, 0, dE, curmask, c->tickets + TICKET_CULL);
+        c->offsets_written = true;
+    }
+}
+
+void launch_offsets(Ctx *c, const EngineDev *dE, const EngineDev &) {
+    DeviceGuard guard(c);
+    if (c->offsets_written) { c->offsets_written = false; return; }
+    launch_pdl(c, "offsets_kernel", offsets_kernel, 1, 1024, 0, dE);
 }
 
 __device__ __forceinline__ int locate_arena(const int *off, int A, int idx) {
@@ -610,6 +717,8 @@
 
 __global__ void __launch_bounds__(256) info_kernel(const EngineDev *gE, unsigned curmask, int kind, int g,
                                                    void *buf, int n_total, int chunks_per_arena) {
+    pdl_wait();
+    pdl_trigger();
     const EngineDev &E = *gE;
     const int *off = E.off + (size_t)g * (E.A + 1);
     const AgentSoA &s = E.grp[g].soa[(curmask >> g) & 1u];
@@ -635,8 +744,7 @@
     const int cap = hE.grp[group].cap;
     const int threads = cap >= 256 ? 256 : ((cap + 31) & ~31);
     const int cpa = (cap + threads - 1) / threads;
-    info_kernel<<<(unsigned)((size_t)hE.A * cpa), threads, 0, c->stream>>>(dE, curmask, kind, group, buf, n_total, cpa);
-    post_launch("info_kernel");
+    launch_pdl(c, "info_kernel", info_kernel, (unsigned)((size_t)hE.A * cpa), threads, 0, dE, curmask, kind, group, buf, n_total, cpa);
 }
 
 __device__ __forceinline__ unsigned long long splitmix64(unsigned long long x) {
@@ -648,6 +756,8 @@
 
 __global__ void __launch_bounds__(256) random_actions_kernel(const EngineDev *gE, unsigned curmask, int g,
                                                              unsigned long long seed, int n_total, int chunks_per_arena) {
+    pdl_wait();
+    pdl_trigger();
     const EngineDev &E = *gE;
     const int *off = E.off + (size_t)g * (E.A + 1);
     const AgentSoA &s = E.grp[g].soa[(curmask >> g) & 1u];
@@ -667,13 +777,15 @@
     const int cap = hE.grp[group].cap;
     const int threads = cap >= 256 ? 256 : ((cap + 31) & ~31);
     const int cpa = (cap + threads - 1) / threads;
-    random_actions_kernel<<<(unsigned)((size_t)hE.A * cpa), threads, 0, c->stream>>>(dE, curmask, group, seed, n_total, cpa);
-    post_launch("random_actions_kernel");
+    launch_pdl(c, "random_actions_kernel", random_actions_kernel, (unsigned)((size_t)hE.A * cpa), threads, 0, dE, curmask, group,
+               seed, n_total, cpa);
 }
 
 __global__ void __launch_bounds__(256) minimap_small_kernel(const EngineDev *gE, unsigned curmask, int og, float *mm_val, int stride) {
     extern __shared__ int hist[];
     __shared__ int counted_s;
+    pdl_wait();
+    pdl_trigger();
     const EngineDev &E = *gE;
     const int ag = blockIdx.x;
     const int a = ag / E.G, j = ag - a * E.G;
@@ -705,6 +817,8 @@
 
 __global__ void __launch_bounds__(256) obs_prepare_kernel(const EngineDev *gE, unsigned curmask, int og, int chunk) {
     extern __shared__ int hist[];
+    pdl_wait();
+    pdl_trigger();
     const EngineDev &E = *gE;
     const int ag = blockIdx.y;
     const int a = ag / E.G, j = ag - a * E.G;
@@ -734,6 +848,8 @@
 }
 
 __global__ void __launch_bounds__(256) minimap_norm_kernel(const EngineDev *gE, int og, float *mm_val, int total, int stride) {
+    pdl_wait();
+    pdl_trigger();
     const EngineDev &E = *gE;
     const int cells = E.grp[og].view_w * E.grp[og].view_h;
     for (int k = blockIdx.x * blockDim.x + threadIdx.x; k < total; k += gridDim.x * blockDim.x) {
@@ -762,20 +878,18 @@
         c->mm_pad_n = need;
     }
     if (cap_max <= 8192 && (size_t)cells * sizeof(int) <= 48 * 1024) {
-        minimap_small_kernel<<<hE.A * hE.G, 256, cells * sizeof(int), c->stream>>>(dE, curmask, og, c->mm_pad, c->mm_stride);
-        post_launch("minimap_small_kernel");
+        launch_pdl(c, "minimap_small_kernel", minimap_small_kernel, hE.A * hE.G, 256, cells * sizeof(int), dE, curmask, og,
+                   c->mm_pad, c->mm_stride);
         return;
     }
     CUDA_CHECK(cudaMemsetAsync(hE.mm_count, 0, (size_t)total * 4, c->stream));
     CUDA_CHECK(cudaMemsetAsync(hE.mm_total, 0, (size_t)hE.A * hE.G * 4, c->stream));
     const int chunk = 4096;
     dim3 grid((cap_max + chunk - 1) / chunk, hE.A * hE.G);
-    obs_prepare_kernel<<<grid, 256, cells * sizeof(int), c->stream>>>(dE, curmask, og, chunk);
-    post_launch("obs_prepare_kernel");
+    launch_pdl(c, "obs_prepare_kernel", obs_prepare_kernel, grid, 256, cells * sizeof(int), dE, curmask, og, chunk);
     int g2 = (total + 255) / 256;
     if (g2 > 8 * g_sms) g2 = 8 * g_sms;
-    minimap_norm_kernel<<<g2, 256, 0, c->stream>>>(dE, og, c->mm_pad, total, c->mm_stride);
-    post_launch("minimap_norm_kernel");
+    launch_pdl(c, "minimap_norm_kernel", minimap_norm_kernel, g2, 256, 0, dE, og, c->mm_pad, total, c->mm_stride);
 }
 
 #ifndef OBS_TA_N
@@ -834,6 +948,8 @@
 __global__ void __launch_bounds__(256) obs_headers_kernel(ObsParams P, int4 *hdr, int chunks_per_arena) {
     extern __shared__ __align__(16) unsigned char hdr_smem[];
     T *rows = (T *)hdr_smem;
+    pdl_wait();
+    pdl_trigger();
     const int a = blockIdx.x / chunks_per_arena;
     const int i0 = (blockIdx.x - a * chunks_per_arena) * blockDim.x;
     const int o0 = P.off[a], n_a = P.off[a + 1] - o0;
@@ -888,8 +1004,7 @@
 #endif
 template <typename T, int NIT, bool TURN>
 __global__ void __launch_bounds__(32 * ObsOut<T>::TA, OBS_MIN_CTAS * OBS_TA_N / ObsOut<T>::TA)
-obs_render_kernel(const __grid_constant__ ObsParams P) {
-    const int n_total = min(P.n_total, __ldg(P.off + P.A));
+obs_render_kernel(const __grid_constant__ ObsParams P, unsigned long long *ts) {
     constexpr int OBS_TA = ObsOut<T>::TA;
     constexpr int OBS_THREADS = 32 * OBS_TA;
     extern __shared__ __align__(128) unsigned char smem_raw[];
@@ -928,8 +1043,12 @@
         }
         if (lane == 0) n_in_s = k;
     }
+    pdl_wait();
+    pdl_trigger();
+    if (ts && threadIdx.x == 0) atomicMin(ts, globaltimer_ns());
     __syncthreads();
     const int n_in = n_in_s;
+    const int n_total = min(P.n_total, __ldg(P.off + P.A));
     const int n_tiles = (n_total + OBS_TA - 1) / OBS_TA;
     constexpr bool LUT_REGS = NIT <= 4 && !TURN;
     int2 lreg[LUT_REGS ? NIT : 1];
@@ -1096,7 +1215,10 @@
 #pragma unroll
         for (int it = 0; it < NIT; ++it) kind[it] = kind1[it];
     }
-    if (threadIdx.x == 0) asm volatile("cp.async.bulk.wait_group 0;" ::: "memory");
+    if (threadIdx.x == 0) {
+        asm volatile("cp.async.bulk.wait_group 0;" ::: "memory");
+        if (ts) atomicMax(ts + 1, globaltimer_ns());
+    }
 }
 
 template <typename T, int NIT, bool TURN>
@@ -1122,8 +1244,7 @@
         const size_t hsm = (size_t)threads * P.F * sizeof(T);
         if (hsm > 48 * 1024) mg::fatal("feature row too long for the header kernel (%d elements)", P.F);
         const int cpa = (P.cap + threads - 1) / threads;
-        obs_headers_kernel<T><<<(unsigned)((size_t)P.A * cpa), threads, hsm, c->stream>>>(P, c->obs_hdr, cpa);
-        post_launch("obs_headers_kernel");
+        launch_pdl(c, "obs_headers_kernel", obs_headers_kernel<T>, (unsigned)((size_t)P.A * cpa), threads, hsm, P, c->obs_hdr, cpa);
     }
     if (headers_only) return;
     Ctx::ObsCfg &cfg = c->obs_cfg[cfg_slot];
@@ -1139,12 +1260,8 @@
     if (P.chunk < 1) P.chunk = 1;
     const int max_chunk = sizeof(T) == 2 ? 2 * OBS_CHUNK : OBS_CHUNK;
     if (P.chunk > max_chunk) P.chunk = max_chunk;
-    cudaEvent_t e0 = nullptr, e1 = nullptr;
-    const bool timed = c->profile && !c->capturing;
-    if (timed) { profile_pair(c, &e0, &e1); CUDA_CHECK(cudaEventRecord(e0, c->stream)); }
-    obs_render_kernel<T, NIT, TURN><<<grid, THREADS, smem, c->stream>>>(P);
-    post_launch("obs_render_kernel");
-    if (timed) CUDA_CHECK(cudaEventRecord(e1, c->stream));
+    unsigned long long *ts = c->profile && !c->capturing ? profile_slot(c) : nullptr;
+    launch_pdl(c, "obs_render_kernel", obs_render_kernel<T, NIT, TURN>, grid, THREADS, smem, P, ts);
 }
 
 static void fill_obs_params(Ctx *c, const EngineDev &hE, const ObsArgs &O, const float *mm_val, int n_total, ObsParams &P) {
@@ -1195,17 +1312,6 @@
     launch_obs_dispatch(c, hE, O, P, n_total, true, false);
 }
 
-__global__ void __launch_bounds__(256) done_reduce_kernel(const EngineDev *gE, int *out) {
-    __shared__ int all_s;
-    if (threadIdx.x == 0) all_s = 1;
-    __syncthreads();
-    int all = 1;
-    for (int a = threadIdx.x; a < gE->A; a += blockDim.x) all &= gE->done[a] & 1;
-    if (!all) all_s = 0;
-    __syncthreads();
-    if (threadIdx.x == 0) *out = all_s;
-}
-
 void read_done(Ctx *c, const EngineDev &hE, int *done_words) {
     no_capture(c, "env_step with a host `done`");
     DeviceGuard guard(c);
@@ -1230,16 +1336,16 @@
     CUDA_CHECK(cudaMemcpyAsync(c->pin_counts, dev_off, n_ints * sizeof(int), cudaMemcpyDeviceToHost, c->stream));
     CUDA_CHECK(cudaEventRecord(c->ev_counts, c->stream));
 }
+void launch_done_to_device(Ctx *c, const EngineDev *dE, const EngineDev &, int *dev_done) {
+    DeviceGuard guard(c);
+    if (c->done_written == dev_done) { c->done_written = nullptr; return; }
+    launch_pdl(c, "done_reduce_kernel", done_reduce_kernel, 1, 256, 0, dE, dev_done);
+}
+
 const int *counts_fetch_wait(Ctx *c) {
     DeviceGuard guard(c);
     CUDA_CHECK(cudaEventSynchronize(c->ev_counts));
     return c->pin_counts;
-}
-
-void launch_done_to_device(Ctx *c, const EngineDev *dE, const EngineDev &, int *dev_done) {
-    DeviceGuard guard(c);
-    done_reduce_kernel<<<1, 256, 0, c->stream>>>(dE, dev_done);
-    post_launch("done_reduce_kernel");
 }
 
 __global__ void __launch_bounds__(256) obs_wire_kernel(const __grid_constant__ ObsParams P, WireHdr *whdr, WireMark *slots,
@@ -1278,6 +1384,8 @@
         }
         if (lane == 0) n_in_s = k;
     }
+    pdl_wait();
+    pdl_trigger();
     __syncthreads();
     const int n_in = n_in_s;
     const int warps = gridDim.x * (blockDim.x >> 5);
@@ -1317,6 +1425,8 @@
 
 __global__ void __launch_bounds__(1024) wire_scan_kernel(const int *chunk_total, long long *base, int n_chunks) {
     __shared__ long long carry_s;
+    pdl_wait();
+    pdl_trigger();
     if (threadIdx.x == 0) carry_s = 0;
     __syncthreads();
     for (int tile = 0; tile < n_chunks; tile += blockDim.x) {
@@ -1338,6 +1448,8 @@
     __shared__ int off_s[WIRE_CHUNK];
     __shared__ unsigned short cnt_s[WIRE_CHUNK];
     const int lane = threadIdx.x & 31, warp = threadIdx.x >> 5, nw = blockDim.x >> 5;
+    pdl_wait();
+    pdl_trigger();
     for (int ch = blockIdx.x; ch < n_chunks; ch += gridDim.x) {
         const int o0 = ch * WIRE_CHUNK, cnt_obs = min(WIRE_CHUNK, n_total - o0);
         int running = 0;
@@ -1401,10 +1513,8 @@
         if (smem > 48 * 1024) mg::fatal("view too large for the wire kernel (%zu bytes of shared memory)", smem);
         int grid = (n_total + 7) / 8;
         if (grid > 8 * c->sms) grid = 8 * c->sms;
-        obs_wire_kernel<<<grid, 256, smem, c->stream>>>(P, c->wire_hdr, c->wire_slots, n_in, c->wire_chunk_total);
-        post_launch("obs_wire_kernel");
-        wire_scan_kernel<<<1, 1024, 0, c->stream>>>(c->wire_chunk_total, c->wire_base, n_chunks);
-        post_launch("wire_scan_kernel");
+        launch_pdl(c, "obs_wire_kernel", obs_wire_kernel, grid, 256, smem, P, c->wire_hdr, c->wire_slots, n_in, c->wire_chunk_total);
+        launch_pdl(c, "wire_scan_kernel", wire_scan_kernel, 1, 1024, 0, (const int *)c->wire_chunk_total, c->wire_base, n_chunks);
     }
     grow_pinned(c, c->h_wire_base, c->h_wire_base_n, (size_t)n_chunks + 1);
     CUDA_CHECK(cudaMemcpyAsync(c->h_wire_base, c->wire_base, ((size_t)n_chunks + 1) * sizeof(long long), cudaMemcpyDeviceToHost, c->stream));
@@ -1420,8 +1530,8 @@
     grow_pinned(c, c->h_wire_marks, c->h_wire_marks_n, (size_t)total_marks + 1);
     {
         int grid = n_chunks < 8 * c->sms ? n_chunks : 8 * c->sms;
-        wire_compact_kernel<<<grid, 256, 0, c->stream>>>(c->wire_hdr, c->wire_slots, n_in, c->wire_base, c->wire_stream, n_total, n_chunks);
-        post_launch("wire_compact_kernel");
+        launch_pdl(c, "wire_compact_kernel", wire_compact_kernel, grid, 256, 0, (const WireHdr *)c->wire_hdr,
+                   (const WireMark *)c->wire_slots, n_in, (const long long *)c->wire_base, c->wire_stream, n_total, n_chunks);
     }
     CUDA_CHECK(cudaEventRecord(c->ev_wire, c->stream));
     CUDA_CHECK(cudaStreamWaitEvent(c->copy, c->ev_wire, 0));
diff --git a/magent_b200/csrc/dev_types.h b/magent_b200/csrc/dev_types.h
--- a/magent_b200/csrc/dev_types.h
+++ b/magent_b200/csrc/dev_types.h
@@ -166,6 +166,7 @@
     int record_events;
     int n_order;
     int order[MG_MAX_GROUPS];
+    int *done_out;
 };
 
 struct ObsArgs {
diff --git a/magent_b200/csrc/engine.cc b/magent_b200/csrc/engine.cc
--- a/magent_b200/csrc/engine.cc
+++ b/magent_b200/csrc/engine.cc
@@ -971,10 +971,11 @@
     S.record_events = first_render_ ? 0 : 1;
     S.n_order = (int)order_.size();
     for (int k = 0; k < S.n_order; ++k) S.order[k] = order_[k];
+    S.done_out = be::is_device_ptr(done) ? done : nullptr;
     be::launch_step(bx_, dE_, hE_, S, max_agents_per_arena());
     ++state_version_;
     order_.clear();
-    if (be::is_device_ptr(done)) {
+    if (S.done_out) {
         be::launch_done_to_device(bx_, dE_, hE_, done);
         may_have_dead_ = true;
         done_stale_ = true;
diff --git a/profiles/probes/probe_pdl_event.cu b/profiles/probes/probe_pdl_event.cu
--- /dev/null
+++ b/profiles/probes/probe_pdl_event.cu
@@ -0,0 +1,62 @@
+#include <cstdio>
+#include <cuda_runtime.h>
+
+__device__ unsigned long long now_ns() {
+    unsigned long long t;
+    asm volatile("mov.u64 %0, %%globaltimer;" : "=l"(t));
+    return t;
+}
+
+__global__ void kernel_a(unsigned long long *ts) {
+    asm volatile("griddepcontrol.launch_dependents;" ::: "memory");
+    const unsigned long long t0 = now_ns();
+    while (now_ns() - t0 < 50000) {}
+    if (threadIdx.x == 0) atomicMax(ts + 0, now_ns());
+}
+
+__global__ void kernel_b(unsigned long long *ts) {
+    if (threadIdx.x == 0) atomicMin(ts + 1, now_ns());
+    asm volatile("griddepcontrol.wait;" ::: "memory");
+}
+
+int main() {
+    cudaStream_t s;
+    cudaStreamCreate(&s);
+    cudaEvent_t ev;
+    cudaEventCreate(&ev);
+    unsigned long long *ts;
+    cudaMalloc(&ts, 2 * sizeof(unsigned long long));
+    cudaLaunchAttribute attr;
+    attr.id = cudaLaunchAttributeProgrammaticStreamSerialization;
+    attr.val.programmaticStreamSerializationAllowed = 1;
+    cudaLaunchConfig_t cfg = {};
+    cfg.gridDim = 4;
+    cfg.blockDim = 128;
+    cfg.stream = s;
+    cfg.attrs = &attr;
+    cfg.numAttrs = 1;
+    for (int with_event = 0; with_event < 2; ++with_event) {
+        long long gap_min = 1ll << 62, gap_max = -(1ll << 62);
+        for (int rep = 0; rep < 20; ++rep) {
+            const unsigned long long init[2] = {0ull, ~0ull};
+            cudaMemcpy(ts, init, sizeof init, cudaMemcpyHostToDevice);
+            cudaLaunchKernelEx(&cfg, kernel_a, ts);
+            if (with_event) cudaEventRecord(ev, s);
+            cudaLaunchKernelEx(&cfg, kernel_b, ts);
+            unsigned long long h[2];
+            cudaMemcpyAsync(h, ts, sizeof h, cudaMemcpyDeviceToHost, s);
+            cudaStreamSynchronize(s);
+            const long long gap = (long long)(h[1] - h[0]);
+            gap_min = gap < gap_min ? gap : gap_min;
+            gap_max = gap > gap_max ? gap : gap_max;
+        }
+        printf("%s: B start - A end = %lld .. %lld ns over 20 runs (%s)\n", with_event ? "event between" : "no event     ",
+               gap_min, gap_max, gap_max < 0 ? "edge kept" : "edge dropped");
+    }
+    cudaError_t e = cudaGetLastError();
+    if (e != cudaSuccess) { printf("CUDA error: %s\n", cudaGetErrorString(e)); return 1; }
+    cudaFree(ts);
+    cudaEventDestroy(ev);
+    cudaStreamDestroy(s);
+    return 0;
+}
```

New measurement: 843.0 million (median of 6 runs). 0.964x the previous value.
